# WU-CVGL/CasualHDRSplat

Hardware: AMD Instinct MI355X
Metric: train-step images/sec (fwd+bwd raster) @ 1M Gaussians 1080p (higher is better)
Workload: dtype f32; 1 GPU; c3: 1000000 Gaussians, 1920x1080, SH degree 3, HDR radiance + CRF tone-map, 1 pose(s)/view, 1 view(s)/step (one per GPU); num_rendered_R=6777809, R_prime=3025699, pixel_pair_evals_E=559372855, seed=0, binning=sync-free fixed capacity 1.25*R, launch=eager (one enqueue per kernel)

## Files before the change

### casualhdrsplat_amd/csrc/api.hip

```cpp
#include <stdarg.h>
#include <stdio.h>
#include <stdlib.h>
#include <string.h>
#include <time.h>
#include <unistd.h>
#include <atomic>

#include "hs_cloud.h"

namespace hs {

static thread_local char g_err[512] = "";

#ifdef HS_TESTING
int fault_injection() {
    static const int mode = [] {
        const char* e = getenv("HS_FAULT_INJECT");
        return (e && !strcmp(e, "sort_ticket")) ? 1 : (e && !strcmp(e, "stalled_chain")) ? 2 : (e && !strcmp(e, "late_block")) ? 3 : 0;
    }();
    return mode;
}
#endif

static std::atomic<int> g_sort_tickets{0};
#ifndef HS_TUNE_DEPTH_MSD_DEFAULT
#define HS_TUNE_DEPTH_MSD_DEFAULT 1
#endif
static std::atomic<int> g_depth_sort{-1};
#ifndef HS_TUNE_HIER_DEFAULT
#define HS_TUNE_HIER_DEFAULT 1
#endif

static int resolve_sorts(const hs_fwd_args& a, SortChoice* c) {
    if (a.tile_sort < 0 || a.tile_sort > HS_TILE_SORT_HIER || a.depth_sort < 0 || a.depth_sort > HS_DEPTH_SORT_COUNT ||
        a.chain_order < 0 || a.chain_order > HS_CHAIN_TICKETS || a.emission_scan < 0 || a.emission_scan > HS_EMISSION_SCAN_INSIDE ||
        a.depth_range_cap < 0 || a.depth_dist_max < -1) {
        set_error("hs_forward: sort selection out of range (tile_sort=%d depth_sort=%d chain_order=%d emission_scan=%d "
                  "depth_range_cap=%d depth_dist_max=%d; see hs_fwd_args in hdrsplat.h)", a.tile_sort, a.depth_sort,
                  a.chain_order, a.emission_scan, a.depth_range_cap, a.depth_dist_max);
        return HS_EINVAL;
    }
    const hs_dims& d = a.dims;
    const int64_t I = (int64_t)d.P * d.n_poses;
    const int64_t gx = (d.W + kTile - 1) / kTile, gy = (d.H + kTile - 1) / kTile;
    const bool can_count = HS_TUNE_COUNT_SORT && count_sort_fits(I, gx * gy * d.n_poses, d.capacity);
    const bool can_hier = hier_fits(I, gx, gy, d.n_poses, d.capacity);
    if (a.tile_sort == HS_TILE_SORT_RADIX) c->tile_sort = kTileSortRadix;
    else if (a.tile_sort == HS_TILE_SORT_HIER && can_hier) c->tile_sort = kTileSortHier;
    else if (a.tile_sort == HS_TILE_SORT_COUNT) c->tile_sort = can_count ? kTileSortCount : kTileSortRadix;
    else if (can_count) c->tile_sort = kTileSortCount;
    else c->tile_sort = (HS_TUNE_HIER_DEFAULT && can_hier) ? kTileSortHier : kTileSortRadix;
    if (!depth_msd_fits(I) || a.depth_sort == HS_DEPTH_SORT_PASSES) c->depth_sort = kDepthSortLsd;
    else if (a.depth_sort == HS_DEPTH_SORT_COUNT) c->depth_sort = kDepthSortMsd;
    else {
        const int v = g_depth_sort.load(std::memory_order_relaxed);
        c->depth_sort = v >= 0 ? v : (HS_TUNE_DEPTH_MSD_DEFAULT ? kDepthSortMsd : kDepthSortLsd);
    }
    c->tickets = a.chain_order ? a.chain_order == HS_CHAIN_TICKETS : g_sort_tickets.load(std::memory_order_relaxed) != 0;
    c->scan_in_emission = a.emission_scan ? a.emission_scan == HS_EMISSION_SCAN_INSIDE : (I >= (2 << 20) && !c->tickets);
    c->range_cap = a.depth_range_cap == 0 ? kMsdCap : (a.depth_range_cap < 64 ? 64 : (a.depth_range_cap > kMsdCap ? kMsdCap : a.depth_range_cap));
    c->dist_max = a.depth_dist_max == 0 ? 16 : (a.depth_dist_max < 0 ? 0 : (a.depth_dist_max > 16 ? 16 : a.depth_dist_max));
    return HS_OK;
}

static uint32_t frame_tag_seed() {
    uint64_t x = (uint64_t)getpid() * 0x9E3779B97F4A7C15ull ^ (uint64_t)time(nullptr) * 0xBF58476D1CE4E5B9ull;
    x ^= x >> 31; x *= 0x94D049BB133111EBull; x ^= x >> 29;
    return (uint32_t)x | 0x80000000u;
}
static std::atomic<uint32_t> g_frame_tag{frame_tag_seed()};
static uint32_t next_frame_tag() {
    uint32_t t;
    do { t = g_frame_tag.fetch_add(1u, std::memory_order_relaxed) + 1u; } while (t == 0u);
    return t;
}

void set_error(const char* fmt, ...) {
    va_list ap;
    va_start(ap, fmt);
    vsnprintf(g_err, sizeof g_err, fmt, ap);
    va_end(ap);
}

int64_t crf_partial_floats(int K, int64_t HW, int n_poses);
int64_t pose_partial_floats(int P, int N);

static int plan(const hs_dims& d, hs_sizes* sz, hs_layout* L) {
    if (d.P < 0 || d.W <= 0 || d.H <= 0 || d.n_poses < 1 || d.capacity < 0 || d.M < 0 || d.crf_K < 0 || d.crf_K > 4096 ||
        d.crf_K == 1 || d.n_poses > kMaxPoses) {
        set_error("hs_plan: bad dims P=%d W=%d H=%d N=%d capacity=%lld", d.P, d.W, d.H, d.n_poses, (long long)d.capacity);
        return HS_EINVAL;
    }
    if (d.n_frames < 0 || d.n_frames > d.n_poses || (d.n_frames > 1 && d.n_poses % d.n_frames != 0)) {
        set_error("hs_plan: n_frames=%d must lie in [0, n_poses=%d] and divide n_poses", d.n_frames, d.n_poses);
        return HS_EINVAL;
    }
    const int F = frames_of(d), npf = d.n_poses / F;
    const int64_t I = (int64_t)d.P * d.n_poses;
    const int64_t gx = (d.W + kTile - 1) / kTile, gy = (d.H + kTile - 1) / kTile;
    const int64_t vtiles = gx * gy * d.n_poses;
    if (I >= (1ll << 30) || vtiles >= (1ll << 31) || d.capacity >= (1ll << 30) || gx * gy >= (1ll << 22)) {
        set_error("hs_plan: problem too large (instances and binning capacity must stay below 2^30, tiles per pose below 2^22)");
        return HS_EINVAL;
    }
    const int64_t HW = (int64_t)d.W * d.H;
    hs_layout l;
    int64_t o = 0;
    auto carve = [&o](int64_t bytes) { int64_t at = o; o = align_up(o + bytes, 256); return at; };
    l.counters = carve(sizeof(hs_counters));
    l.rec = carve(I * kRecFloats * 4);
    l.depth = carve(I * 4);
    l.radii = carve(I * 4);
    l.tiles_touched = carve(I * 4);
    l.offsets = carve(I * 4);
    l.cov3D = carve((int64_t)d.P * 6 * 4);
    l.clamped = carve(I);
    l.scan_spine = carve(((I + 255) / 256 + 1) * 4);
    l.binfo = carve(I * 8);
    sz->geom_bytes = o;
    o = 0;
    l.keys_sorted = carve(2 * align_up(d.capacity * 4, 256));
    l.point_list = l.keys_sorted + align_up(d.capacity * 4, 256);
    l.pairs_tmp = carve(d.capacity * 8);
    l.ranges = carve(vtiles * 8);
    l.sort_tmp = carve(sort_tmp_bytes(I));
    l.depth_ws = carve(depth_ws_words(I) * 4);
    l.depth_pairs = carve(2 * I * 8);
    l.inst_sorted = carve(I * 4);
    l.offs_sorted = carve(I * 4);
    l.pair_sort_tmp = carve(emit_scan_words(I) * 4 + sort_tmp_bytes(d.capacity));
    l.pair_flags = carve(d.capacity);
    l.pair_act = carve(d.capacity);
    l.tile_matrix = carve(count_matrix_words(I, vtiles, d.capacity) * 4);
    l.hier_ws = carve(hier_ws_words(I, gx, gy, d.n_poses, d.capacity) * 4);
    sz->binning_bytes = o;
    o = 0;
    l.final_T = carve(HW * d.n_poses * 4);
    l.n_contrib = carve(HW * d.n_poses * 4);
    l.pose_hdr = carve(HW * 3 * 4 * (d.n_poses + (npf > 1 ? F : 0)));
    l.tile_work = carve(vtiles * 4);
    l.tile_order = carve(vtiles * 4);
    sz->image_bytes = o;
    o = 0;
    l.pair_grads = carve(d.capacity * kPairFloats * 4);
    l.crf_partials = carve(crf_partial_floats(d.crf_K, HW, d.n_poses) * 4);
    l.inst_grads = carve(I * kInstFloats * 4);
    l.pose_partials = carve(pose_partial_floats(d.P, d.n_poses) * 4);
    sz->bwd_bytes = o;
    if (L) *L = l;
    return HS_OK;
}

static int debug_sync(int flags, hipStream_t s, const char* stage) {
    if (!(flags & HS_FLAG_DEBUG)) return HS_OK;
    const hipError_t e = hipStreamSynchronize(s);
    if (e != hipSuccess) {
        set_error("debug: stage `%s` failed: %s", stage, hipGetErrorString(e));
        return HS_EHIP;
    }
    return HS_OK;
}

static int check_common(const hs_dims& d, const float* means3D, const float* shs, const float* colors,
                        const float* scales, const float* rots, const float* cov, const float* view,
                        const float* proj, const float* campos, const float* bg, const char* who) {
    if (!means3D || !view || !proj || !campos || !bg) { set_error("%s: null required pointer", who); return HS_EINVAL; }
    if ((shs == nullptr) == (colors == nullptr)) { set_error("%s: provide exactly one of shs / colors_precomp", who); return HS_EINVAL; }
    const bool sr = scales && rots;
    if (sr == (cov != nullptr) || ((scales == nullptr) != (rots == nullptr))) {
        set_error("%s: provide exactly one of (scales, rotations) / cov3D_precomp", who);
        return HS_EINVAL;
    }
    if (shs) {
        if (d.M > 32) {
            set_error("%s: M=%d SH coefficients per channel; at most 32 are supported", who, d.M);
            return HS_EINVAL;
        }
        if (d.sh_degree < 0 || d.sh_degree > 3 || (d.sh_degree + 1) * (d.sh_degree + 1) > d.M) {
            set_error("%s: sh_degree %d needs %d coefficients, M=%d", who, d.sh_degree, (d.sh_degree + 1) * (d.sh_degree + 1), d.M);
            return HS_EINVAL;
        }
    }
    if (rots && ((uintptr_t)rots & 15)) { set_error("%s: rotations must be 16-byte aligned", who); return HS_EINVAL; }
    return HS_OK;
}

static int check_flags(int flags, const char* who) {
    if ((flags & HS_FLAG_RADIANCE_EXP) && (flags & HS_FLAG_RADIANCE_SOFTPLUS)) {
        set_error("%s: HS_FLAG_RADIANCE_EXP and HS_FLAG_RADIANCE_SOFTPLUS are mutually exclusive", who);
        return HS_EINVAL;
    }
    return HS_OK;
}

static int check_loss_shape(int32_t planes, int32_t H, int32_t W, float lambda, const char* who) {
    if (planes < 1 || H < 1 || W < 1 || (int64_t)planes * H * W >= (1ll << 31)) {
        set_error("%s: bad shape planes=%d H=%d W=%d (each >= 1, planes * H * W < 2^31)", who, planes, H, W);
        return HS_EINVAL;
    }
    if (!(lambda >= 0.0f && lambda <= 1.0f)) {
        set_error("%s: lambda_dssim=%g outside [0, 1]", who, (double)lambda);
        return HS_EINVAL;
    }
    return HS_OK;
}

static int check_activate_tensor(const char* who, const char* name, const void* key, const void* const* need, const char* const* need_names, int n) {
    if (!key) return HS_OK;
    if (check_aligned(who, key, name, 4)) return HS_EINVAL;
    for (int i = 0; i < n; ++i) {
        if (!need[i]) { set_error("%s: %s is given but %s is NULL", who, name, need_names[i]); return HS_EINVAL; }
        if (check_aligned(who, need[i], need_names[i], 4)) return HS_EINVAL;
    }
    return HS_OK;
}

}

using namespace hs;

extern "C" {

int hs_version(void) { return HS_VERSION; }

const char* hs_last_error(void) { return g_err; }

int hs_plan(const hs_dims* dims, hs_sizes* sizes, hs_layout* layout) {
    if (!dims || !sizes) { set_error("hs_plan: null argument"); return HS_EINVAL; }
    return plan(*dims, sizes, layout);
}

int hs_max_frames(void) { return kMaxPoses; }

#ifdef HS_TESTING
HS_API uint32_t hs_test_next_frame_tag(void) {
    const uint32_t t = g_frame_tag.load(std::memory_order_relaxed) + 1u;
    return t == 0u ? 1u : t;
}
#endif

int hs_forward(const hs_fwd_args* a, void* hip_stream) {
    if (!a) { set_error("hs_forward: null args"); return HS_EINVAL; }
    hipStream_t s = (hipStream_t)hip_stream;
    hs_sizes sz; hs_layout L;
    int rc = plan(a->dims, &sz, &L);
    if (rc) return rc;
    if ((rc = check_flags(a->flags, "hs_forward"))) return rc;
    SortChoice sort;
    if ((rc = resolve_sorts(*a, &sort))) return rc;
    if (a->dims.P > 0) {
        rc = check_common(a->dims, a->means3D, a->shs, a->colors_precomp, a->scales, a->rotations, a->cov3D_precomp,
                          a->viewmatrices, a->projmatrices, a->camposes, a->bg, "hs_forward");
        if (rc) return rc;
        if (!a->opacities || ((a->stages & HS_STAGE_PREPROCESS) && !a->radii)) {
            set_error("hs_forward: null opacities/radii");
            return HS_EINVAL;
        }
    }
    if (!a->geom || !a->bg) { set_error("hs_forward: null geom/bg"); return HS_EINVAL; }
    if ((a->flags & HS_FLAG_HDR) && (!a->exposure || !a->crf_table || a->crf_K < 2 || a->crf_K > 4096 || !(a->crf_umax > a->crf_umin))) {
        set_error("hs_forward: HDR needs exposure, crf_table, 2 <= crf_K <= 4096 and umax > umin");
        return HS_EINVAL;
    }
    if ((a->flags & HS_FLAG_HDR) && a->dims.crf_K != a->crf_K) {
        set_error("hs_forward: dims.crf_K (%d, sizes the workspaces) differs from crf_K (%d)", a->dims.crf_K, a->crf_K);
        return HS_EINVAL;
    }
    if (((uintptr_t)a->geom & 255) || ((uintptr_t)a->binning & 255) || ((uintptr_t)a->image & 255)) {
        set_error("hs_forward: workspaces must be 256-byte aligned");
        return HS_EINVAL;
    }
    if (a->dims.P == 0) {
        const int64_t gx0 = (a->dims.W + kTile - 1) / kTile, gy0 = (a->dims.H + kTile - 1) / kTile;
        const bool bin = (a->stages & HS_STAGE_BIN) && !(a->stages & HS_STAGE_PREPROCESS_ONLY) && a->binning;
        rc = launch_empty_frame((a->stages & HS_STAGE_PREPROCESS) ? (hs_counters*)((char*)a->geom + L.counters) : nullptr,
                                bin ? (uint2*)((char*)a->binning + L.ranges) : nullptr, gx0 * gy0 * a->dims.n_poses,
                                bin ? (uint32_t*)a->counters_host : nullptr, (const hs_counters*)((char*)a->geom + L.counters), s);
        if (rc) return rc;
    }
    const uint32_t frame_tag = ((a->stages & HS_STAGE_PREPROCESS) && (a->stages & HS_STAGE_BIN) && a->binning) ? next_frame_tag() : 0u;
    if ((a->stages & HS_STAGE_PREPROCESS) && a->dims.P > 0) {
        rc = launch_preprocess_fwd(*a, L, s, frame_tag);
        if (rc) return rc;
        if ((rc = debug_sync(a->flags, s, "preprocess"))) return rc;
        if (!(a->stages & HS_STAGE_BIN)) {
            rc = launch_scan(*a, L, s);
            if (rc) return rc;
        }
    }
    if ((a->stages & HS_STAGE_BIN) && !(a->stages & HS_STAGE_PREPROCESS_ONLY)) {
        if (!a->binning) { set_error("hs_forward: null binning workspace"); return HS_EINVAL; }
        if (a->dims.P > 0) {
            rc = launch_binning(*a, L, sort, s, frame_tag);
            if (rc) return rc;
            if ((rc = debug_sync(a->flags, s, "binning"))) return rc;
        }
    }
    if ((a->stages & HS_STAGE_OFFSETS) && a->dims.P > 0) {
        rc = launch_scan(*a, L, s);
        if (rc) return rc;
        if ((rc = launch_cov3d(*a, L, s))) return rc;
        if (a->binning && a->dims.capacity > 0)
            if ((rc = launch_tile_keys(*a, L, s))) return rc;
    }
    if (a->stages & HS_STAGE_RENDER) {
        if (!a->binning || !a->image || !a->out_color) { set_error("hs_forward: null binning/image/out_color"); return HS_EINVAL; }
        rc = launch_render_fwd(*a, L, s);
        if (rc) return rc;
        if ((rc = debug_sync(a->flags, s, "render forward"))) return rc;
    }
    return HS_OK;
}

int hs_backward(const hs_bwd_args* a, void* hip_stream) {
    if (!a) { set_error("hs_backward: null args"); return HS_EINVAL; }
    hipStream_t s = (hipStream_t)hip_stream;
    hs_sizes sz; hs_layout L;
    int rc = plan(a->dims, &sz, &L);
    if (rc) return rc;
    if ((rc = check_flags(a->flags, "hs_backward"))) return rc;
    if (frames_of(a->dims) > 1 && (a->dL_dout_alpha || a->dL_dout_invdepth)) {
        set_error("hs_backward: dL_dout_alpha / dL_dout_invdepth are per-image gradients and are not supported with n_frames=%d",
                  a->dims.n_frames);
        return HS_EINVAL;
    }
    rc = check_common(a->dims, a->means3D, a->shs, a->colors_precomp, a->scales, a->rotations, a->cov3D_precomp,
                      a->viewmatrices, a->projmatrices, a->camposes, a->bg, "hs_backward");
    if (rc) return rc;
    if (!a->geom || !a->binning || !a->image || !a->bwd || !a->dL_dout_color) {
        set_error("hs_backward: null workspace or dL_dout_color");
        return HS_EINVAL;
    }
    if ((a->flags & HS_FLAG_HDR) && (!a->exposure || !a->crf_table || a->crf_K < 2 || a->crf_K > 4096 || a->dims.crf_K != a->crf_K)) {
        set_error("hs_backward: HDR needs exposure, crf_table and dims.crf_K == crf_K");
        return HS_EINVAL;
    }
    const int npose_out = (a->dL_dviewmatrices != nullptr) + (a->dL_dprojmatrices != nullptr) + (a->dL_dcamposes != nullptr);
    if (npose_out != 0 && npose_out != 3) {
        set_error("hs_backward: pose gradients need dL_dviewmatrices, dL_dprojmatrices and dL_dcamposes together");
        return HS_EINVAL;
    }
    const int ndens = (a->densify_grad_accum != nullptr) + (a->densify_denom != nullptr) + (a->densify_max_radii != nullptr);
    if (ndens != 0 && ndens != 3) {
        set_error("hs_backward: densification statistics need grad_accum, denom and max_radii together");
        return HS_EINVAL;
    }
    if (a->g_begin != 0 || a->g_end != 0) {
        if (a->g_begin < 0 || a->g_end < a->g_begin || a->g_end > a->dims.P || (a->g_begin & 127) ||
            (a->stages & ~HS_BWD_PROJECT)) {
            set_error("hs_backward: [g_begin, g_end) = [%d, %d) needs 0 <= g_begin <= g_end <= P, g_begin a multiple of 128, "
                      "and stages == HS_BWD_PROJECT", a->g_begin, a->g_end);
            return HS_EINVAL;
        }
    }
    if (a->dims.P == 0) return HS_OK;
    const bool crf_in_tail = HS_TUNE_CRF_IN_RENDER_TAIL && (a->stages & HS_BWD_RENDER) && (a->stages & HS_BWD_CRF) &&
                             !(a->flags & HS_FLAG_DEBUG) && a->crf_K <= 1024;
    if (a->stages & HS_BWD_RENDER) {
        rc = launch_render_bwd(*a, L, s, nullptr, nullptr, crf_in_tail);
        if (rc) return rc;
        if ((rc = debug_sync(a->flags, s, "render backward"))) return rc;
    }
    CrfReduce crf_reduce{nullptr, 0, 0, 0, nullptr, nullptr, 0};
    const bool sums_follow = (a->stages & (HS_BWD_PREPROCESS | HS_BWD_SEGSUM)) != 0 && !(a->flags & HS_FLAG_DEBUG);
    if (a->stages & HS_BWD_CRF) {
        rc = launch_crf_bwd(*a, L, s, sums_follow ? &crf_reduce : nullptr, crf_in_tail);
        if (rc) return rc;
        if ((rc = debug_sync(a->flags, s, "CRF gradient"))) return rc;
    }
    if (a->stages & (HS_BWD_PREPROCESS | HS_BWD_SEGSUM | HS_BWD_PROJECT)) {
        const bool whole = (a->stages & HS_BWD_PREPROCESS) != 0;
        rc = launch_preprocess_bwd(*a, L, s, whole || (a->stages & HS_BWD_SEGSUM), whole || (a->stages & HS_BWD_PROJECT),
                                   crf_reduce.nblocks ? &crf_reduce : nullptr);
        if (rc) return rc;
        if ((rc = debug_sync(a->flags, s, "preprocess backward"))) return rc;
    }
    return HS_OK;
}

int hs_depth_sort(int mode) {
    if (mode >= 0) hs::g_depth_sort.store(mode ? 1 : 0, std::memory_order_relaxed);
    const int v = hs::g_depth_sort.load(std::memory_order_relaxed);
    return v >= 0 ? v : (HS_TUNE_DEPTH_MSD_DEFAULT ? 1 : 0);
}

int hs_sort_tickets(int enable) {
    if (enable >= 0) hs::g_sort_tickets.store(enable ? 1 : 0, std::memory_order_relaxed);
    return hs::g_sort_tickets.load(std::memory_order_relaxed);
}

int hs_mark_visible(int32_t P, const float* means3D, const float* viewmatrix, uint8_t* visible, void* hip_stream) {
    if (P < 0 || (P > 0 && (!means3D || !viewmatrix || !visible))) { set_error("hs_mark_visible: bad argument"); return HS_EINVAL; }
    if (P == 0) return HS_OK;
    return launch_mark_visible(P, means3D, viewmatrix, visible, (hipStream_t)hip_stream);
}

int hs_sh_backward_views(int32_t P, int32_t M, int32_t sh_degree, int32_t V, const float* means3D, const float* camposes,
                         const float* dL_dview_colors, float* dL_dshs, void* hip_stream) {
    if (P < 0 || V < 1 || sh_degree < 0 || sh_degree > 3 || M < (sh_degree + 1) * (sh_degree + 1) || M > 16 ||
        (P > 0 && (!means3D || !camposes || !dL_dview_colors || !dL_dshs))) {
        set_error("hs_sh_backward_views: bad argument");
        return HS_EINVAL;
    }
    if (P == 0) return HS_OK;
    return launch_sh_backward_views(P, M, sh_degree, V, means3D, camposes, dL_dview_colors, dL_dshs, (hipStream_t)hip_stream);
}

int hs_spline_poses(int32_t n_knots, int32_t n_times, int32_t kind, const float* delta, const float* base_w2c,
                    const float* times, float* w2c, float* jacobian, int32_t* segment, void* hip_stream) {
    if (n_times < 0 || (kind != 0 && kind != 1) || n_knots < (kind == 1 ? 4 : 2) ||
        (n_times > 0 && (!delta || !base_w2c || !times || !w2c || !jacobian || !segment))) {
        set_error("hs_spline_poses: bad argument (kind 0 = linear needs >= 2 knots, 1 = cubic >= 4)");
        return HS_EINVAL;
    }
    if (n_times == 0) return HS_OK;
    return launch_spline_poses(n_knots, n_times, kind, delta, base_w2c, times, w2c, jacobian, segment, (hipStream_t)hip_stream);
}

int hs_render_stats(const hs_fwd_args* fwd, const hs_bwd_args* bwd, uint64_t* stats, uint64_t* bwd_timeline, void* hip_stream) {
    if ((!fwd && !bwd) || !stats) { set_error("hs_render_stats: null argument"); return HS_EINVAL; }
    hipStream_t s = (hipStream_t)hip_stream;
    hs_sizes sz; hs_layout L;
    if (fwd) {
        int rc = plan(fwd->dims, &sz, &L);
        if (rc) return rc;
        if (!fwd->geom || !fwd->binning || !fwd->image || !fwd->out_color || !fwd->bg) {
            set_error("hs_render_stats: forward args need geom/binning/image/out_color/bg");
            return HS_EINVAL;
        }
        if (fwd->dims.P > 0 && (rc = launch_render_fwd(*fwd, L, s, (unsigned long long*)stats))) return rc;
    }
    if (bwd) {
        int rc = plan(bwd->dims, &sz, &L);
        if (rc) return rc;
        if (!bwd->geom || !bwd->binning || !bwd->image || !bwd->bwd || !bwd->dL_dout_color || !bwd->bg) {
            set_error("hs_render_stats: backward args need geom/binning/image/bwd/dL_dout_color/bg");
            return HS_EINVAL;
        }
        if (bwd->dims.P > 0 && (rc = launch_render_bwd(*bwd, L, s, (unsigned long long*)stats, (unsigned long long*)bwd_timeline))) return rc;
    }
    return HS_OK;
}

int64_t hs_loss_workspace_bytes(int32_t planes, int32_t H, int32_t W, int32_t with_partials) {
    if (check_loss_shape(planes, H, W, 0.0f, "hs_loss_workspace_bytes")) return HS_EINVAL;
    const int64_t pairs = align_up(loss_pair_count(planes, H, W) * 16, 256);
    return pairs + (with_partials ? (int64_t)12 * planes * H * W : 0);
}

int hs_photometric_loss(const hs_loss_args* a, void* hip_stream) {
    if (!a) { set_error("hs_photometric_loss: null args"); return HS_EINVAL; }
    int rc = check_loss_shape(a->planes, a->H, a->W, a->lambda_dssim, "hs_photometric_loss");
    if (rc) return rc;
    if (!a->image || !a->target || !a->workspace || !a->out) {
        set_error("hs_photometric_loss: null image/target/workspace/out");
        return HS_EINVAL;
    }
    if ((uintptr_t)a->workspace & 255) { set_error("hs_photometric_loss: workspace must be 256-byte aligned"); return HS_EINVAL; }
    return launch_loss_fwd(*a, (hipStream_t)hip_stream);
}

int hs_photometric_loss_backward(const hs_loss_args* a, void* hip_stream) {
    if (!a) { set_error("hs_photometric_loss_backward: null args"); return HS_EINVAL; }
    int rc = check_loss_shape(a->planes, a->H, a->W, a->lambda_dssim, "hs_photometric_loss_backward");
    if (rc) return rc;
    if (!a->image || !a->target || !a->partials || !a->dL_dloss || !a->dL_dimage) {
        set_error("hs_photometric_loss_backward: null image/target/partials/dL_dloss/dL_dimage");
        return HS_EINVAL;
    }
    return launch_loss_bwd(*a, (hipStream_t)hip_stream);
}

int hs_activate(const hs_activate_args* a, void* hip_stream) {
    const char* who = "hs_activate";
    if (check_args(who, a) || check_rows(who, "P", a->P)) return HS_EINVAL;
    int rc;
    if (a->P == 0) return HS_OK;
    const void* o[] = {a->opacities}; const char* on[] = {"opacities"};
    const void* s[] = {a->scales}; const char* sn[] = {"scales"};
    const void* r[] = {a->rotations}; const char* rn[] = {"rotations"};
    if ((rc = check_activate_tensor(who, "opacity_raw", a->opacity_raw, o, on, 1))) return rc;
    if ((rc = check_activate_tensor(who, "scales_raw", a->scales_raw, s, sn, 1))) return rc;
    if ((rc = check_activate_tensor(who, "rotations_raw", a->rotations_raw, r, rn, 1))) return rc;
    return launch_activate_fwd(*a, (hipStream_t)hip_stream);
}

int hs_activate_backward(const hs_activate_args* a, void* hip_stream) {
    const char* who = "hs_activate_backward";
    if (check_args(who, a) || check_rows(who, "P", a->P)) return HS_EINVAL;
    int rc;
    if (a->g_begin < 0 || a->g_begin > a->g_end || a->g_end > a->P) {
        set_error("%s: rows [g_begin=%lld, g_end=%lld) are not inside [0, P=%lld]", who, (long long)a->g_begin, (long long)a->g_end,
                  (long long)a->P);
        return HS_EINVAL;
    }
    if (a->g_begin == a->g_end) return HS_OK;
    const void* o[] = {a->opacities}; const char* on[] = {"opacities"};
    const void* s[] = {a->scales}; const char* sn[] = {"scales"};
    const void* r[] = {a->rotations, a->rotations_raw}; const char* rn[] = {"rotations", "rotations_raw"};
    if ((rc = check_activate_tensor(who, "dL_dopacities", a->dL_dopacities, o, on, 1))) return rc;
    if ((rc = check_activate_tensor(who, "dL_dscales", a->dL_dscales, s, sn, 1))) return rc;
    if ((rc = check_activate_tensor(who, "dL_drotations", a->dL_drotations, r, rn, 2))) return rc;
    return launch_activate_bwd(*a, (hipStream_t)hip_stream);
}

int64_t hs_sort_tmp_bytes(int64_t n) { return sort_tmp_bytes(n) + 256 + 2 * align_up(n * 8, 256) + 2 * align_up(n * 4, 256); }

int hs_sort_pairs(const uint64_t* keys_in, const uint32_t* vals_in, uint64_t* keys_out, uint32_t* vals_out,
                  int64_t n, int32_t nbits, void* tmp, void* hip_stream) {
    if (n < 0 || n >= (1ll << 30) || nbits < 1 || nbits > 64 || (n > 0 && (!keys_in || !vals_in || !keys_out || !vals_out || !tmp))) {
        set_error("hs_sort_pairs: bad argument");
        return HS_EINVAL;
    }
    if (n == 0) return HS_OK;
    hipStream_t s = (hipStream_t)hip_stream;
    char* t = (char*)tmp;
    uint32_t* n_dev = (uint32_t*)t;
    uint32_t* fail_word = n_dev + 1; t += 256;
    uint64_t* kb = (uint64_t*)t; t += align_up(n * 8, 256);
    uint32_t* vb = (uint32_t*)t; t += align_up(n * 4, 256);
    uint64_t* ka = (uint64_t*)t; t += align_up(n * 8, 256);
    uint32_t* va = (uint32_t*)t; t += align_up(n * 4, 256);
    HS_HIP_CHECK(hipMemsetD32Async((hipDeviceptr_t)n_dev, (int)(uint32_t)n, 1, s));
    HS_HIP_CHECK(hipMemsetD32Async((hipDeviceptr_t)fail_word, 0, 1, s));
    HS_HIP_CHECK(hipMemcpyAsync(ka, keys_in, (size_t)n * 8, hipMemcpyDeviceToDevice, s));
    HS_HIP_CHECK(hipMemcpyAsync(va, vals_in, (size_t)n * 4, hipMemcpyDeviceToDevice, s));
    int rc = launch_radix_sort(ka, va, kb, vb, n_dev, n, nbits, t, fail_word, s);
    if (rc) return rc;
    const bool in_a = sort_passes(nbits) % 2 == 0;
    HS_HIP_CHECK(hipMemcpyAsync(keys_out, in_a ? ka : kb, (size_t)n * 8, hipMemcpyDeviceToDevice, s));
    HS_HIP_CHECK(hipMemcpyAsync(vals_out, in_a ? va : vb, (size_t)n * 4, hipMemcpyDeviceToDevice, s));
    return HS_OK;
}

}
```

### casualhdrsplat_amd/csrc/hs_common.h

```cpp
#pragma once
#include <hip/hip_runtime.h>
#include <stdint.h>

#include "../../include/hdrsplat.h"

#if defined(__HIP_DEVICE_COMPILE__) && !defined(__gfx950__)
#error "libhdrsplat is written for gfx950 (MI355X) only: build with --offload-arch=gfx950"
#endif

namespace hs {

void set_error(const char* fmt, ...);

#define HS_HIP_CHECK(expr)                                                                         \
    do {                                                                                           \
        hipError_t e_ = (expr);                                                                    \
        if (e_ != hipSuccess) {                                                                    \
            ::hs::set_error("%s failed: %s (%s:%d)", #expr, hipGetErrorString(e_), __FILE__, __LINE__); \
            return HS_EHIP;                                                                        \
        }                                                                                          \
    } while (0)
#define HS_LAUNCH_CHECK() HS_HIP_CHECK(hipGetLastError())

#ifndef HS_TUNE_CRF_IN_RENDER_TAIL
#define HS_TUNE_CRF_IN_RENDER_TAIL 1
#endif

#ifndef HS_TUNE_COUNT_SORT
#define HS_TUNE_COUNT_SORT 1
#endif

constexpr int kTile = HS_TILE;
constexpr int kRecF4 = 4;
constexpr int kPairF4 = 4;
constexpr int kInstF4 = 4;
constexpr int kRecFloats = 4 * kRecF4;
constexpr int kPairFloats = 4 * kPairF4;
constexpr int kInstFloats = 4 * kInstF4;
constexpr int kSortBlock = 256;
constexpr int kDepthBins = 512, kDepthDigitBits = 9;
#ifndef HS_TUNE_DEPTH_ITEMS
#define HS_TUNE_DEPTH_ITEMS 8
#endif
constexpr int kDepthSortItems = HS_TUNE_DEPTH_ITEMS, kDepthSortLook = 8;
constexpr int kPairSortItems = 16, kPairSortLook = 8;
constexpr int kU64SortItems = 16;
constexpr int kDepthTile = kDepthSortItems * kDepthBins, kPairTile = kPairSortItems * kSortBlock, kU64Tile = kU64SortItems * kSortBlock;
static_assert(kPairTile == kU64Tile && kDepthTile >= kPairTile, "the scratch of every sort is sized for the smallest tile");
constexpr int kSortTileMin = kPairTile;

static inline int64_t align_up(int64_t v, int64_t a) { return (v + a - 1) / a * a; }
static inline int ceil_div(int64_t a, int64_t b) { return (int)((a + b - 1) / b); }
constexpr int kMaxPoses = 21845;
static inline int frames_of(const hs_dims& d) { return d.n_frames > 1 ? d.n_frames : 1; }

static inline int tile_bits(uint32_t n) {
    int b = 0;
    while (n) { ++b; n >>= 1; }
    return b;
}

int launch_preprocess_fwd(const hs_fwd_args& a, const hs_layout& L, hipStream_t s, uint32_t frame_tag);
int launch_scan(const hs_fwd_args& a, const hs_layout& L, hipStream_t s);
int launch_cov3d(const hs_fwd_args& a, const hs_layout& L, hipStream_t s);
struct SortChoice;
int launch_binning(const hs_fwd_args& a, const hs_layout& L, const SortChoice& sort, hipStream_t s, uint32_t frame_tag);
int launch_empty_frame(hs_counters* clear, uint2* ranges, int64_t ntiles, uint32_t* counters_host, const hs_counters* counters,
                       hipStream_t s);
int launch_render_fwd(const hs_fwd_args& a, const hs_layout& L, hipStream_t s, unsigned long long* stats = nullptr);
int launch_render_bwd(const hs_bwd_args& a, const hs_layout& L, hipStream_t s, unsigned long long* stats = nullptr,
                      unsigned long long* timeline = nullptr, bool crf_in_tail = false);
int render_stats_count();
struct CrfReduce;
int launch_crf_bwd(const hs_bwd_args& a, const hs_layout& L, hipStream_t s, CrfReduce* defer, bool in_render_tail = false);
int launch_preprocess_bwd(const hs_bwd_args& a, const hs_layout& L, hipStream_t s, bool segsum, bool project,
                          const CrfReduce* crf_reduce);
int launch_mark_visible(int P, const float* means3D, const float* view, uint8_t* vis, hipStream_t s);
int launch_spline_poses(int J, int T, int kind, const float* delta, const float* base, const float* times, float* w2c,
                        float* jac, int* seg, hipStream_t s);
int launch_sh_backward_views(int P, int M, int deg, int V, const float* means3D, const float* camposes,
                             const float* view_colors, float* d_shs, hipStream_t s);
int64_t loss_pair_count(int planes, int H, int W);
int launch_loss_fwd(const hs_loss_args& a, hipStream_t s);
int launch_loss_bwd(const hs_loss_args& a, hipStream_t s);
int launch_activate_fwd(const hs_activate_args& a, hipStream_t s);
int launch_activate_bwd(const hs_activate_args& a, hipStream_t s);

constexpr int kGhistCopies = 16;
constexpr int kGhistWords = kGhistCopies * 8 * 256;
constexpr int kTicketWords = 128, kDepthBitsAt = 32, kDepthBitsCopies = 16, kDepthBitsWords = 4 * kDepthBitsCopies;
static_assert(kDepthBitsAt >= 8 && kDepthBitsAt % 2 == 0 && kDepthBitsAt + kDepthBitsWords <= kTicketWords, "depth bits live in the ticket row");
__host__ __device__ inline int64_t sweep_pass_words(int64_t nblk, int bins = 256) { return nblk * bins; }
static inline int64_t sort_scratch_words(int64_t n, int passes, int tile, int bins = 256) {
    return n > 0 ? kGhistWords + kTicketWords + (int64_t)passes * sweep_pass_words((n + tile - 1) / tile, bins) : 0;
}
static inline int64_t depth_scratch_words(int64_t I) { return sort_scratch_words(I, 4, kDepthTile, kDepthBins); }
int64_t sort_tmp_bytes(int64_t n);
constexpr int kMsdBits = 12, kMsdBuckets = 1 << kMsdBits;
#ifndef HS_TUNE_MSD_RANGE
#define HS_TUNE_MSD_RANGE 2048
#endif
constexpr int kMsdRange = HS_TUNE_MSD_RANGE, kMsdCap = 4096;
#ifndef HS_TUNE_MSD_SMALL_RANGE
#define HS_TUNE_MSD_SMALL_RANGE 512
#endif
static inline int depth_msd_range(int64_t I) { return I <= (1 << 18) ? HS_TUNE_MSD_SMALL_RANGE : kMsdRange; }
static inline bool depth_msd_fits(int64_t I) { return I > 0 && I < (2 << 20); }
static inline int depth_msd_tile(int64_t I) { return I <= (1 << 18) ? 1024 : 4096; }
static inline int64_t depth_msd_rows(int64_t I) { return (I + depth_msd_tile(I) - 1) / depth_msd_tile(I); }
static inline int64_t depth_ws_words(int64_t I) {
    return depth_msd_fits(I) ? depth_msd_rows(I) * (kMsdBuckets / 2 + kMsdBuckets + 1) + kMsdBuckets : 0;
}
enum DepthSort { kDepthSortLsd = 0, kDepthSortMsd = 1 };
static inline int64_t emit_scan_words(int64_t I) { return 2 * ((I + 255) / 256 + 2) / 64 * 64 + 64; }
static inline int64_t pair_scratch_words(int64_t I, int64_t capacity, int passes) {
    return emit_scan_words(I) + sort_scratch_words(capacity, passes, kPairSortItems * kSortBlock);
}
int launch_radix_sort(uint64_t* k0, uint32_t* v0, uint64_t* k1, uint32_t* v1, const uint32_t* n_dev,
                      int64_t n_launch, int nbits, void* tmp, uint32_t* fail_word, hipStream_t s, bool zeroed = false);
#ifdef HS_TESTING
int fault_injection();
#else
constexpr int fault_injection() { return 0; }
#endif
static inline int sort_passes(int nbits) { return (nbits + 7) / 8; }
constexpr int kCountTilesMax = 4096;
constexpr int64_t kCountMatrixMax = 1ll << 21;
static inline bool count_sort_fits(int64_t I, int64_t vtiles, int64_t capacity) {
    return capacity > 0 && I > 0 && vtiles <= kCountTilesMax && ((I + 255) / 256) * vtiles <= kCountMatrixMax;
}
static inline int64_t count_matrix_words(int64_t I, int64_t vtiles, int64_t capacity) {
    return count_sort_fits(I, vtiles, capacity) ? 2 * ((I + 255) / 256) * vtiles + vtiles : 0;
}
constexpr int kSuper = 8;
constexpr int kHierStMax = 2048;
constexpr int kHierChunkMin = 512, kHierChunkMax = 1024, kHierRoundsMax = kHierChunkMax / 4 / 64;
static inline int hier_chunk(int64_t I) { return I >= (2ll << 20) ? kHierChunkMax : kHierChunkMin; }
constexpr int kHierCopies = 16;
static inline int64_t hier_super_tiles(int64_t gx, int64_t gy, int64_t n_poses) {
    return ((gx + kSuper - 1) / kSuper) * ((gy + kSuper - 1) / kSuper) * n_poses;
}
static inline bool hier_fits(int64_t I, int64_t gx, int64_t gy, int64_t n_poses, int64_t capacity) {
    return capacity > 0 && I > 0 && hier_super_tiles(gx, gy, n_poses) <= kHierStMax;
}
struct HierWs {
    int64_t nst, chunks_max;
    int64_t st_count, tile_total, zero_words, tile_start, coarse_first, chunk_first, desc, counts, words;
    HierWs(int64_t gx, int64_t gy, int64_t n_poses, int64_t capacity) {
        nst = hier_super_tiles(gx, gy, n_poses);
        chunks_max = (capacity + kHierChunkMin - 1) / kHierChunkMin + nst;
        const int64_t nst_pad = (nst + 63) / 64 * 64;
        int64_t o = 64;
        st_count = o; o += kHierCopies * nst_pad;
        tile_total = o; o += nst * 64;
        zero_words = o;
        tile_start = o; o += nst * 64;
        coarse_first = o; o += nst_pad + 64;
        chunk_first = o; o += nst_pad + 64;
        desc = o; o += chunks_max * 4;
        counts = o; o += chunks_max * 64 * 2;
        words = o;
    }
    int64_t nst_pad() const { return (nst + 63) / 64 * 64; }
};
static inline int64_t hier_ws_words(int64_t I, int64_t gx, int64_t gy, int64_t n_poses, int64_t capacity) {
    return hier_fits(I, gx, gy, n_poses, capacity) ? HierWs(gx, gy, n_poses, capacity).words : 0;
}
enum TileSort { kTileSortRadix = 0, kTileSortCount = 1, kTileSortHier = 2 };
struct SortChoice {
    int tile_sort;
    int depth_sort;
    bool tickets;
    bool scan_in_emission;
    int range_cap;
    int dist_max;
};
int launch_tile_keys(const hs_fwd_args& a, const hs_layout& L, hipStream_t s);

__device__ __forceinline__ void tagged_or(unsigned long long* p, uint32_t tag, uint32_t bits) {
    unsigned long long old = __hip_atomic_load(p, __ATOMIC_RELAXED, __HIP_MEMORY_SCOPE_AGENT);
    for (;;) {
        const unsigned long long cur = (uint32_t)(old >> 32) == tag ? old : ((unsigned long long)tag << 32);
        const unsigned long long nw = cur | bits;
        if (nw == old) return;
        const unsigned long long prev = atomicCAS(p, old, nw);
        if (prev == old) return;
        old = prev;
    }
}
template <int CTRL, int ROW_MASK = 0xF>
__device__ __forceinline__ float dpp_f32(float v) {
    return __int_as_float(__builtin_amdgcn_update_dpp(0, __float_as_int(v), CTRL, ROW_MASK, 0xF, false));
}
__device__ __forceinline__ float wave_sum_hi_f32(float v) {
    v += dpp_f32<0xB1>(v);
    v += dpp_f32<0x4E>(v);
    v += dpp_f32<0x141>(v);
    v += dpp_f32<0x140>(v);
    v += dpp_f32<0x142, 0xA>(v);
    v += dpp_f32<0x143, 0xC>(v);
    return v;
}

struct CrfReduce {
    const float* partials; int bx, planes, K; float* d_table; float* d_exposure;
    int nblocks;
    int F;
};
__device__ __forceinline__ void crf_reduce_block(const CrfReduce& c, int block) {
    const int K = c.K;
    const int i = block * 4 + (threadIdx.x >> 6);
    const int lane = threadIdx.x & 63;
    if (i >= 3 * K + c.F) return;
    const bool expo = i >= 3 * K;
    const int ch = expo ? 0 : i / K, k = expo ? K : i - ch * K;
    float acc = 0.f;
    const int frame_rows = (c.planes / c.F) * c.bx;
    const int nrows = expo ? frame_rows : (c.planes / 3) * c.bx;
    const int row0 = expo ? (i - 3 * K) * frame_rows : 0;
    for (int r = lane; r < nrows; r += 64) {
        const int row = expo ? row0 + r : ((r / c.bx) * 3 + ch) * c.bx + (r % c.bx);
        acc += c.partials[(int64_t)row * (K + 1) + k];
    }
    acc = wave_sum_hi_f32(acc);
    if (lane == 63) {
        if (!expo) { if (c.d_table) c.d_table[i] = acc; }
        else if (c.d_exposure) c.d_exposure[i - 3 * K] = acc;
    }
}

template <int CTRL, int ROW_MASK = 0xF>
__device__ __forceinline__ uint32_t dpp_u32(uint32_t v) {
    return (uint32_t)__builtin_amdgcn_update_dpp(0, (int)v, CTRL, ROW_MASK, 0xF, false);
}
__device__ __forceinline__ uint32_t wave_or_hi(uint32_t v) {
    v |= dpp_u32<0xB1>(v);
    v |= dpp_u32<0x4E>(v);
    v |= dpp_u32<0x141>(v);
    v |= dpp_u32<0x140>(v);
    v |= dpp_u32<0x142, 0xA>(v);
    v |= dpp_u32<0x143, 0xC>(v);
    return v;
}
__device__ __forceinline__ void depth_bits_accumulate2(uint32_t o_in, uint32_t nz_in, unsigned long long* bits, uint32_t tag,
                                                       uint32_t* s_two ) {
    const uint32_t o = wave_or_hi(o_in), nz = wave_or_hi(nz_in);
    if ((threadIdx.x & 63) == 63) { if (o) atomicOr(&s_two[0], o); if (nz) atomicOr(&s_two[1], nz); }
    __syncthreads();
    if (threadIdx.x < 2 && s_two[threadIdx.x])
        tagged_or(bits + 2 * (blockIdx.x % kDepthBitsCopies) + threadIdx.x, tag, s_two[threadIdx.x]);
}
__device__ __forceinline__ void depth_bits_accumulate(uint32_t key, bool visible, unsigned long long* bits, uint32_t tag,
                                                      uint32_t* s_two ) {
    depth_bits_accumulate2(visible ? key : 0u, visible ? ~key : 0u, bits, tag, s_two);
}
__device__ __forceinline__ float radiance_dact(int act, float col, bool was_clamped) {
    if (act == 1) return col;
    if (act == 2) return -expm1f(-col);
    return was_clamped ? 0.f : 1.f;
}

struct SegsumArgs {
    int64_t I;
    const uint32_t* inst_sorted; const uint32_t* offs_sorted;
    const float4* pair_grads; const uint8_t* pair_flags; float4* inst_grads; const hs_counters* counters;
    const int* radii_inst; const uint8_t* clamped; float* view_colors; const float4* rec; int act;
};
__device__ __forceinline__ void pair_segsum_body(const SegsumArgs& a, int64_t t) {
    const int64_t i = t >> 2;
    const int q = (int)(t & 3);
    const bool valid = i < a.I && !a.counters->overflow;
    const uint32_t beg = valid ? (i == 0 ? 0u : a.offs_sorted[i - 1]) : 0u;
    const uint32_t end = valid ? a.offs_sorted[i] : 0u;
    float r[10] = {0.f, 0.f, 0.f, 0.f, 0.f, 0.f, 0.f, 0.f, 0.f, 0.f};
    for (uint32_t s = beg + q; s < end; s += 8) {
        const bool two = s + 4 < end;
        const bool f0 = a.pair_flags[s] != 0;
        const bool f1 = two && a.pair_flags[s + 4] != 0;
        float4 a0 = make_float4(0.f, 0.f, 0.f, 0.f), a1 = a0, b0 = a0, b1 = a0;
        float2 a2 = make_float2(0.f, 0.f), b2 = a2;
        if (f0) {
            a0 = a.pair_grads[kPairF4 * (int64_t)s + 0];
            a1 = a.pair_grads[kPairF4 * (int64_t)s + 1];
            a2 = reinterpret_cast<const float2*>(a.pair_grads + kPairF4 * (int64_t)s + 2)[0];
        }
        if (f1) {
            b0 = a.pair_grads[kPairF4 * (int64_t)(s + 4) + 0];
            b1 = a.pair_grads[kPairF4 * (int64_t)(s + 4) + 1];
            b2 = reinterpret_cast<const float2*>(a.pair_grads + kPairF4 * (int64_t)(s + 4) + 2)[0];
        }
        r[0] += a0.x; r[1] += a0.y; r[2] += a0.z; r[3] += a0.w;
        r[4] += a1.x; r[5] += a1.y; r[6] += a1.z; r[7] += a1.w;
        r[8] += a2.x; r[9] += a2.y;
        r[0] += b0.x; r[1] += b0.y; r[2] += b0.z; r[3] += b0.w;
        r[4] += b1.x; r[5] += b1.y; r[6] += b1.z; r[7] += b1.w;
        r[8] += b2.x; r[9] += b2.y;
    }
#pragma unroll
    for (int k = 0; k < 10; ++k) {
        r[k] += __shfl_xor(r[k], 1);
        r[k] += __shfl_xor(r[k], 2);
    }
    if (i < a.I && q == 0) {
        const int64_t inst = a.counters->overflow >= 2u ? i : (int64_t)a.inst_sorted[i];
        float4* o = a.inst_grads + kInstF4 * inst;
        o[0] = make_float4(r[0], r[1], r[2], r[3]);
        o[1] = make_float4(r[4], r[5], r[6], r[7]);
        o[2] = make_float4(r[8], r[9], 0.f, 0.f);
        if constexpr (kInstF4 == 4) o[3] = make_float4(0.f, 0.f, 0.f, 0.f);
        if (a.view_colors) {
            const uint8_t cl = a.clamped[inst];
            const bool on = a.radii_inst[inst] > 0;
            float col[3] = {0.f, 0.f, 0.f};
            if (a.act != 0 && on) {
                const float4 rb = a.rec[kRecF4 * inst + 1];
                col[0] = rb.z; col[1] = rb.w; col[2] = reinterpret_cast<const float*>(a.rec + kRecF4 * inst + 2)[0];
            }
            a.view_colors[3 * inst + 0] = on ? radiance_dact(a.act, col[0], cl & 1) * r[6] : 0.f;
            a.view_colors[3 * inst + 1] = on ? radiance_dact(a.act, col[1], cl & 2) * r[7] : 0.f;
            a.view_colors[3 * inst + 2] = on ? radiance_dact(a.act, col[2], cl & 4) * r[8] : 0.f;
        }
    }
}

__device__ __forceinline__ float xform_row(const float* m, int i, float x, float y, float z) {
    return ((m[i] * x + m[4 + i] * y) + m[8 + i] * z) + m[12 + i];
}

}
```

### casualhdrsplat_amd/csrc/render.hip

```cpp
#include "hs_common.h"

namespace hs {

namespace {

constexpr float kAlphaMin = 1.0f / 255.0f;
constexpr float kAlphaMax = 0.99f;
constexpr float kTmin = 0.0001f;
constexpr float kLogEps = 1e-8f;


enum {
    kStBwdTrips = 0,
    kStBwdEmpty = 1,
    kStBwdActivePix = 2,
    kStBwdCulled = 3,
    kStBwdHist = 4,
    kStBwdStaged = 10,
    kStBwdBatches = 11,
    kStFwdTrips = 12, kStFwdEmpty = 13, kStFwdActivePix = 14, kStFwdCulled = 15, kStFwdStaged = 16, kStFwdBatches = 17,
    kStCount = 24
};
struct WaveStats {
    unsigned long long v[kStCount];
    __device__ __forceinline__ void clear() {
#pragma unroll
        for (int i = 0; i < kStCount; ++i) v[i] = 0;
    }
    __device__ __forceinline__ void flush(unsigned long long* dst) const {
        if ((threadIdx.x & 63) == 0) {
#pragma unroll
            for (int i = 0; i < kStCount; ++i)
                if (v[i]) atomicAdd(dst + i, v[i]);
        }
    }
};

template <int CTRL, int ROW_MASK = 0xF>
__device__ __forceinline__ float dpp(float v) {
    return __int_as_float(__builtin_amdgcn_update_dpp(0, __float_as_int(v), CTRL, ROW_MASK, 0xF, false));
}
__device__ __forceinline__ float wave_sum_hi(float v) {
    v += dpp<0xB1>(v);
    v += dpp<0x4E>(v);
    v += dpp<0x141>(v);
    v += dpp<0x140>(v);
    v += dpp<0x142, 0xA>(v);
    v += dpp<0x143, 0xC>(v);
    return v;
}
__device__ __forceinline__ float halve16(float x, float y) {
    auto r = __builtin_amdgcn_permlane16_swap(__float_as_uint(x), __float_as_uint(y), false, false);
    return __uint_as_float(r[0]) + __uint_as_float(r[1]);
}
template <bool TEN>
__device__ __forceinline__ void reduce_in_rows(const float* g, float g9, float& w0, float& w1, float& w2) {
    float z0, z1, z2, z3, z4;
    if constexpr (TEN) {
        asm("s_nop 1\n\t"
            "v_add_f32_dpp %3, %9, %9 row_shr:8 row_mask:0xf bank_mask:0xc\n\t"
            "v_add_f32_dpp %3, %8, %8 row_shl:8 row_mask:0xf bank_mask:0x3\n\t"
            "v_add_f32_dpp %4, %11, %11 row_shr:8 row_mask:0xf bank_mask:0xc\n\t"
            "v_add_f32_dpp %4, %10, %10 row_shl:8 row_mask:0xf bank_mask:0x3\n\t"
            "v_add_f32_dpp %5, %13, %13 row_shr:8 row_mask:0xf bank_mask:0xc\n\t"
            "v_add_f32_dpp %5, %12, %12 row_shl:8 row_mask:0xf bank_mask:0x3\n\t"
            "v_add_f32_dpp %6, %15, %15 row_shr:8 row_mask:0xf bank_mask:0xc\n\t"
            "v_add_f32_dpp %6, %14, %14 row_shl:8 row_mask:0xf bank_mask:0x3\n\t"
            "v_add_f32_dpp %7, %17, %17 row_shr:8 row_mask:0xf bank_mask:0xc\n\t"
            "v_add_f32_dpp %7, %16, %16 row_shl:8 row_mask:0xf bank_mask:0x3\n\t"
            "v_add_f32_dpp %0, %4, %4 row_shr:4 row_mask:0xf bank_mask:0xa\n\t"
            "v_add_f32_dpp %0, %3, %3 row_shl:4 row_mask:0xf bank_mask:0x5\n\t"
            "v_add_f32_dpp %1, %6, %6 row_shr:4 row_mask:0xf bank_mask:0xa\n\t"
            "v_add_f32_dpp %1, %5, %5 row_shl:4 row_mask:0xf bank_mask:0x5\n\t"
            "v_add_f32_dpp %2, %7, %7 row_shr:4 row_mask:0xf bank_mask:0xa\n\t"
            "v_add_f32_dpp %2, %7, %7 row_shl:4 row_mask:0xf bank_mask:0x5\n\t"
            "s_nop 1"
            : "=&v"(w0), "=&v"(w1), "=&v"(w2), "=&v"(z0), "=&v"(z1), "=&v"(z2), "=&v"(z3), "=&v"(z4)
            : "v"(g[0]), "v"(g[1]), "v"(g[2]), "v"(g[3]), "v"(g[4]), "v"(g[5]), "v"(g[6]), "v"(g[7]), "v"(g[8]), "v"(g9));
    } else {
        asm("s_nop 1\n\t"
            "v_add_f32_dpp %3, %9, %9 row_shr:8 row_mask:0xf bank_mask:0xc\n\t"
            "v_add_f32_dpp %3, %8, %8 row_shl:8 row_mask:0xf bank_mask:0x3\n\t"
            "v_add_f32_dpp %4, %11, %11 row_shr:8 row_mask:0xf bank_mask:0xc\n\t"
            "v_add_f32_dpp %4, %10, %10 row_shl:8 row_mask:0xf bank_mask:0x3\n\t"
            "v_add_f32_dpp %5, %13, %13 row_shr:8 row_mask:0xf bank_mask:0xc\n\t"
            "v_add_f32_dpp %5, %12, %12 row_shl:8 row_mask:0xf bank_mask:0x3\n\t"
            "v_add_f32_dpp %6, %15, %15 row_shr:8 row_mask:0xf bank_mask:0xc\n\t"
            "v_add_f32_dpp %6, %14, %14 row_shl:8 row_mask:0xf bank_mask:0x3\n\t"
            "v_add_f32_dpp %7, %16, %16 row_ror:8 row_mask:0xf bank_mask:0xf\n\t"
            "v_add_f32_dpp %0, %4, %4 row_shr:4 row_mask:0xf bank_mask:0xa\n\t"
            "v_add_f32_dpp %0, %3, %3 row_shl:4 row_mask:0xf bank_mask:0x5\n\t"
            "v_add_f32_dpp %1, %6, %6 row_shr:4 row_mask:0xf bank_mask:0xa\n\t"
            "v_add_f32_dpp %1, %5, %5 row_shl:4 row_mask:0xf bank_mask:0x5\n\t"
            "v_add_f32_dpp %2, %7, %7 row_ror:4 row_mask:0xf bank_mask:0xf\n\t"
            "s_nop 1"
            : "=&v"(w0), "=&v"(w1), "=&v"(w2), "=&v"(z0), "=&v"(z1), "=&v"(z2), "=&v"(z3), "=&v"(z4)
            : "v"(g[0]), "v"(g[1]), "v"(g[2]), "v"(g[3]), "v"(g[4]), "v"(g[5]), "v"(g[6]), "v"(g[7]), "v"(g[8]));
    }
}
__device__ __forceinline__ float reduce_in_quads(float t) {
    asm("s_nop 1\n\t"
        "v_add_f32_dpp %0, %0, %0 quad_perm:[1,0,3,2] row_mask:0xf bank_mask:0xf\n\t"
        "s_nop 1\n\t"
        "v_add_f32_dpp %0, %0, %0 quad_perm:[2,3,0,1] row_mask:0xf bank_mask:0xf"
        : "+v"(t));
    return t;
}

template <bool TEN>
__device__ __forceinline__ void group_reduce(const float* g, float g9, int xor16_addr, float& t0, float& t1) {
    float w0, w1, w2;
    reduce_in_rows<TEN>(g, g9, w0, w1, w2);
    const float u0 = halve16(w0, w1);
    const float u1 = w2 + __int_as_float(__builtin_amdgcn_ds_bpermute(xor16_addr, __float_as_int(w2)));
    t0 = reduce_in_quads(u0);
    t1 = reduce_in_quads(u1);
}

__device__ __forceinline__ int mask_prefix(uint64_t m) {
    return (int)__builtin_amdgcn_mbcnt_hi((uint32_t)(m >> 32), __builtin_amdgcn_mbcnt_lo((uint32_t)m, 0u));
}

__device__ __forceinline__ uint32_t wave_max_u32(uint32_t v) {
#pragma unroll
    for (int d = 32; d >= 1; d >>= 1) v = max(v, (uint32_t)__shfl_xor((int)v, d));
    return v;
}

struct Crf {
    const float* table;
    int K;
    float umin, umax, dt;
};

__device__ __forceinline__ void crf_locate(const Crf& c, float Hv, int& i, float& f, float& xv, bool& interior) {
    xv = Hv * c.dt;
    const float u = __logf(fmaxf(xv, kLogEps));
    float s = (u - c.umin) / (c.umax - c.umin) * (float)(c.K - 1);
    bool in = true;
    if (!(s > 0.f)) { s = 0.f; in = false; }
    if (s >= (float)(c.K - 1)) { s = (float)(c.K - 1); in = false; }
    i = (int)floorf(s);
    if (i > c.K - 2) i = c.K - 2;
    f = s - (float)i;
    interior = in && (xv > kLogEps);
}
__device__ __forceinline__ float crf_eval(const Crf& c, int ch, float Hv) {
    int i; float f, xv; bool in;
    crf_locate(c, Hv, i, f, xv, in);
    const float* t = c.table + ch * c.K;
    return t[i] * (1.f - f) + t[i + 1] * f;
}
__device__ __forceinline__ float crf_grad_H(const Crf& c, int ch, float Hv, float g) {
    int i; float f, xv; bool in;
    crf_locate(c, Hv, i, f, xv, in);
    if (!in) return 0.f;
    const float* t = c.table + ch * c.K;
    const float scale = (float)(c.K - 1) / (c.umax - c.umin);
    return g * (t[i + 1] - t[i]) * scale / xv * c.dt;
}

constexpr float kLog2e = 1.4426950408889634f;

typedef float f2 __attribute__((ext_vector_type(2)));

#ifndef HS_NO_OPSEL_ASM
__device__ __forceinline__ f2 pk_fma_hi(f2 pair, f2 w, f2 acc) {
    asm("v_pk_fma_f32 %0, %1, %2, %0 op_sel:[1,0,0] op_sel_hi:[1,1,1]" : "+v"(acc) : "v"(pair), "v"(w));
    return acc;
}
__device__ __forceinline__ f2 pk_mul_hi(f2 pair, f2 w) {
    f2 r;
    asm("v_pk_mul_f32 %0, %1, %2 op_sel:[1,0] op_sel_hi:[1,1]" : "=v"(r) : "v"(pair), "v"(w));
    return r;
}
#else
__device__ __forceinline__ f2 pk_fma_hi(f2 pair, f2 w, f2 acc) { return acc + f2{pair.y, pair.y} * w; }
__device__ __forceinline__ f2 pk_mul_hi(f2 pair, f2 w) { return f2{pair.y, pair.y} * w; }
#endif

__device__ __forceinline__ void scale_entry(float4& a, float4& b) {
    a.z *= -0.5f * kLog2e; a.w *= -kLog2e; b.x *= -0.5f * kLog2e;
}

template <int WIDTH>
__device__ __forceinline__ bool block_may_touch(const float4 a, const float4 b, float sx, float sy) {
    const float A2 = a.z, B2 = a.w, C2 = b.x, o = b.y;
    if (!(o >= kAlphaMin)) return false;
    if (!(A2 < 0.f && C2 < 0.f && 4.f * A2 * C2 - B2 * B2 > 0.f)) return true;
    const float thr = -(__log2f(255.f * o) * 1.0001f + 0.05f);
    const float dx_lo = a.x - (sx + (float)(WIDTH - 1)), dx_hi = a.x - sx, dy_lo = a.y - (sy + 7.f), dy_hi = a.y - sy;
    const float dx_e = fminf(fmaxf(0.f, dx_lo), dx_hi);
    const float dy_e = fminf(fmaxf(0.f, dy_lo), dy_hi);
    const float dy_s = fminf(fmaxf(-0.5f * B2 * dx_e / C2, dy_lo), dy_hi);
    const float dx_s = fminf(fmaxf(-0.5f * B2 * dy_e / A2, dx_lo), dx_hi);
    const float p1 = dx_e * (A2 * dx_e + B2 * dy_s) + C2 * dy_s * dy_s;
    const float p2 = dx_s * (A2 * dx_s + B2 * dy_e) + C2 * dy_e * dy_e;
    return fmaxf(p1, p2) >= thr;
}

__device__ __forceinline__ void lane_pixels(int lane, int sx, int sy, int& px, int& py0) {
    px = sx + 8 * (lane >> 5) + (lane & 7);
    py0 = sy + 2 * ((lane >> 3) & 3);
}

struct RenderFwd {
    int W, H, gx, ntiles, N, flags;
    const uint2* ranges; const uint32_t* point_list; const float4* rec; const float* bg;
    float* out_color; float* out_hdr; float* final_T; uint32_t* n_contrib; float* pose_hdr;
    float* out_invdepth;
    Crf crf;
    const float* exposure;
    unsigned long long* stats;
    unsigned long long* timeline;
    uint8_t* pair_act;
    uint32_t* tile_work;
};

constexpr int kBatch = 128;

__device__ __forceinline__ int xcd_strip_tile(int b, int nb, int gx) {
    constexpr int kXcd = 8, kRows = 2;
    const int x = b % kXcd, k = b / kXcd;
    const int per = nb / kXcd, rem = nb % kXcd;
    int p = x * per + min(x, rem) + k;
    const int rows = nb / gx;
    const int nstrips = (rows + kRows - 1) / kRows;
    const int strip_tiles = kRows * gx;
    const int last_short = nstrips * strip_tiles - nb;
    int c = 0;
    for (; c < kXcd - 1; ++c) {
        const int ns = (nstrips - c + kXcd - 1) / kXcd;
        const int nt = ns * strip_tiles - (((nstrips - 1) % kXcd) == c ? last_short : 0);
        if (p < nt) break;
        p -= nt;
    }
    const int s_local = p / strip_tiles, r = p - s_local * strip_tiles;
    return (c + kXcd * s_local) * strip_tiles + r;
}

__device__ __forceinline__ float hs_exp2(float x) { return __builtin_amdgcn_exp2f(x); }

struct PixF {
    float T, C0, C1, C2, D;
    uint32_t last;
};
constexpr int kFcmpOGE = 3, kFcmpOLE = 5;
struct PairF {
    f2 T, C0, C1, C2, D;
    uint32_t last0, last1;
};
template <bool DEPTH>
__device__ __forceinline__ uint64_t blend_fwd_pair(PairF& s, uint64_t& done0, uint64_t& done1, f2 pw, f2 alpha, float r,
                                                   float g, float b, float invd, uint32_t idx1, int* n_pixels = nullptr) {
    const uint64_t valid0 = ~done0 & __builtin_amdgcn_fcmpf(pw.x, 0.f, kFcmpOLE) &
                            __builtin_amdgcn_fcmpf(alpha.x, kAlphaMin, kFcmpOGE);
    const uint64_t valid1 = ~done1 & __builtin_amdgcn_fcmpf(pw.y, 0.f, kFcmpOLE) &
                            __builtin_amdgcn_fcmpf(alpha.y, kAlphaMin, kFcmpOGE);
    const f2 one = {1.f, 1.f};
    const f2 test_T = s.T * (one - alpha);
    const uint64_t cont0 = valid0 & __builtin_amdgcn_fcmpf(test_T.x, kTmin, kFcmpOGE);
    const uint64_t cont1 = valid1 & __builtin_amdgcn_fcmpf(test_T.y, kTmin, kFcmpOGE);
    done0 |= valid0 ^ cont0;
    done1 |= valid1 ^ cont1;
    const bool upd0 = __builtin_amdgcn_inverse_ballot_w64(cont0), upd1 = __builtin_amdgcn_inverse_ballot_w64(cont1);
    const f2 aT = alpha * s.T;
    const f2 w = {upd0 ? aT.x : 0.f, upd1 ? aT.y : 0.f};
    const f2 rr = {r, r}, bb = {b, b};
    s.C0 += rr * w; s.C1 = pk_fma_hi(f2{r, g}, w, s.C1); s.C2 += bb * w;
    if constexpr (DEPTH) { const f2 dd = {invd, invd}; s.D += dd * w; }
    s.T = f2{upd0 ? test_T.x : s.T.x, upd1 ? test_T.y : s.T.y};
    s.last0 = upd0 ? idx1 : s.last0;
    s.last1 = upd1 ? idx1 : s.last1;
    if (n_pixels) *n_pixels = __popcll(cont0) + __popcll(cont1);
    return cont0 | cont1;
}

__device__ __forceinline__ void write_pixel_fwd(const RenderFwd& p, const PixF& st, int pose, int px, int py) {
    const int64_t HW = (int64_t)p.H * p.W;
    const int64_t pix = (int64_t)py * p.W + px;
    p.final_T[(int64_t)pose * HW + pix] = st.T;
    p.n_contrib[(int64_t)pose * HW + pix] = st.last;
    const float H0 = st.C0 + st.T * p.bg[0], H1 = st.C1 + st.T * p.bg[1], H2 = st.C2 + st.T * p.bg[2];
    const bool hdr = p.flags & HS_FLAG_HDR;
    if (p.pose_hdr) {
        float* ph = p.pose_hdr + (int64_t)pose * 3 * HW;
        ph[pix] = H0; ph[HW + pix] = H1; ph[2 * HW + pix] = H2;
    }
    if (p.N == 1) {
        float* const oc = p.out_color + (int64_t)pose * 3 * HW;
        if (hdr) {
            Crf c = p.crf;
            c.dt = p.exposure[pose];
            if (p.out_hdr) { float* const oh = p.out_hdr + (int64_t)pose * 3 * HW; oh[pix] = H0; oh[HW + pix] = H1; oh[2 * HW + pix] = H2; }
            oc[pix] = crf_eval(c, 0, H0);
            oc[HW + pix] = crf_eval(c, 1, H1);
            oc[2 * HW + pix] = crf_eval(c, 2, H2);
        } else {
            oc[pix] = H0; oc[HW + pix] = H1; oc[2 * HW + pix] = H2;
        }
    }
}

constexpr int kFwdEntF = 12;

template <bool DEPTH, bool STATS>
__global__ void __launch_bounds__(kBatch) __attribute__((amdgpu_waves_per_eu((DEPTH || STATS) ? 1 : 7)))
render_fwd_kernel(RenderFwd p) {
    constexpr int KB = kBatch;
    constexpr int kEnt = kFwdEntF * 4;
    constexpr int kSentinel = KB * kEnt;
    constexpr int kListLen = KB + 8;
    __shared__ __attribute__((aligned(16))) float s_ent[(KB + 1) * kFwdEntF];
    __shared__ int s_alive[2][2];
    __shared__ uint16_t s_list[2][2][kListLen];
    __shared__ uint8_t s_taken[2][2][KB];
    __shared__ uint32_t s_work[2];

    const int vt = xcd_strip_tile(blockIdx.x, gridDim.x, p.gx);
    const int pose = vt / p.ntiles;
    const int tile = vt - pose * p.ntiles;
    const int tx = tile % p.gx, ty = tile / p.gx;
    const int wave = threadIdx.x >> 6, lane = threadIdx.x & 63;
    const int grp = lane >> 5;
    const int sx = tx * kTile, sy = ty * kTile + wave * 8;
    int px, py0;
    lane_pixels(lane, sx, sy, px, py0);
    const int py1 = py0 + 1;
    const bool in0 = px < p.W && py0 < p.H, in1 = px < p.W && py1 < p.H;
    const float pxf = (float)px;
    const f2 pyf = {(float)py0, (float)py1};
    const float sxf = (float)sx, syf = (float)sy;

    const uint2 range = p.ranges[vt];
    const int n = (int)(range.y - range.x);

    PairF ps;
    ps.T = f2{1.f, 1.f};
    ps.C0 = ps.C1 = ps.C2 = ps.D = f2{0.f, 0.f};
    ps.last0 = ps.last1 = 0;
    uint64_t done0 = __builtin_amdgcn_ballot_w64(!in0), done1 = __builtin_amdgcn_ballot_w64(!in1);

    float4 ra = make_float4(0.f, 0.f, 0.f, 0.f), rb = ra;
    float rcb = 0.f, rdepth = 1.f;
    if ((int)threadIdx.x < n) {
        const uint32_t id = p.point_list[range.x + threadIdx.x];
        const float4* r = p.rec + kRecF4 * (int64_t)id;
        ra = r[0]; rb = r[1]; rcb = reinterpret_cast<const float*>(r + 2)[0];
        if constexpr (DEPTH) rdepth = reinterpret_cast<const float*>(r + 2)[1];
    }
    WaveStats ws;
    if constexpr (STATS) ws.clear();
    const char* const ent = reinterpret_cast<const char*>(s_ent);
    float* const my_ent = s_ent + threadIdx.x * kFwdEntF;
    const uint16_t* const my_list = s_list[wave][grp];
    if (threadIdx.x < kFwdEntF) s_ent[KB * kFwdEntF + threadIdx.x] = 0.f;
    auto flush_activity = [&](int base_prev, int cnt_prev) {
        const int t = threadIdx.x;
        if (t < cnt_prev)
            p.pair_act[(int64_t)range.x + base_prev + t] = (uint8_t)(s_taken[0][0][t] | s_taken[0][1][t] | s_taken[1][0][t] | s_taken[1][1][t]);
        s_taken[0][0][t] = 0; s_taken[0][1][t] = 0; s_taken[1][0][t] = 0; s_taken[1][1][t] = 0;
    };
    auto walk = [&](int i0, int i1, int base48) -> uint32_t {
        uint32_t act_lo = 0u, act_hi = 0u;
        uint32_t pos = 0u;
        const uint32_t npos = (uint32_t)(i1 - i0);
        const uint16_t* lp = my_list + i0;
        auto trip = [&]() {
            const int jb = (int)*lp++;
            const char* e = ent + jb;
            const float4 a = *reinterpret_cast<const float4*>(e);
            const float4 b = *reinterpret_cast<const float4*>(e + 16);
            const float2 c = *reinterpret_cast<const float2*>(e + 32);
            const float dx = a.x - pxf;
            const f2 dy = a.y - pyf;
            const float t = a.z * dx * dx, u = a.w * dx;
            const f2 pw = dy * (b.x * dy + u) + t;
            const float al0 = fminf(kAlphaMax, b.y * hs_exp2(pw.x));
            const float al1 = fminf(kAlphaMax, b.y * hs_exp2(pw.y));
            const uint32_t idx48 = (uint32_t)(base48 + jb + kEnt);
            int n_pix = 0;
            const uint64_t took = blend_fwd_pair<DEPTH>(ps, done0, done1, pw, f2{al0, al1}, b.z, b.w, c.x, DEPTH ? c.y : 0.f, idx48,
                                                        STATS ? &n_pix : nullptr);
            if constexpr (STATS) ws.v[kStFwdActivePix] += n_pix;
#pragma clang diagnostic push
#pragma clang diagnostic ignored "-Winline-asm"
            asm("s_mov_b32 m0, %2\n\t"
                "v_writelane_b32 %0, %3, m0\n\t"
                "v_writelane_b32 %1, %4, m0\n\t"
                "s_add_u32 %2, %2, 1"
                : "+v"(act_lo), "+v"(act_hi), "+s"(pos) : "s"((uint32_t)took), "s"((uint32_t)(took >> 32)) : "scc", "m0");
#pragma clang diagnostic pop
            if constexpr (STATS) { ws.v[kStFwdTrips] += 1; ws.v[kStFwdEmpty] += took == 0ull; }
        };
        if (npos >= 2u) {
            do {
                trip();
                trip();
            } while (pos + 2u <= npos && (done0 & done1) != ~0ull);
        }
        if (pos + 1u == npos && (done0 & done1) != ~0ull) trip();
        return (act_lo != 0u ? 1u : 0u) | (act_hi != 0u ? 4u : 0u);
    };
    s_taken[0][0][threadIdx.x] = 0; s_taken[0][1][threadIdx.x] = 0; s_taken[1][0][threadIdx.x] = 0; s_taken[1][1][threadIdx.x] = 0;
    uint32_t n_taken = 0;
    int it = 0, base = 0;
    for (; base < n; base += KB, ++it) {
        const uint64_t fin = done0 & done1;
        const bool wave_alive = fin != ~0ull;
        if (lane == 0) s_alive[it & 1][wave] = wave_alive;
        __syncthreads();
        if (it > 0) flush_activity(base - KB, KB);
        if (!(s_alive[it & 1][0] | s_alive[it & 1][1])) break;
        const int cnt = min(KB, n - base);
        if constexpr (STATS) { if (wave == 0) { ws.v[kStFwdStaged] += cnt; ws.v[kStFwdBatches] += 1; } }
        if ((int)threadIdx.x < cnt) {
            scale_entry(ra, rb);
            reinterpret_cast<float4*>(my_ent)[0] = ra;
            reinterpret_cast<float4*>(my_ent)[1] = rb;
            reinterpret_cast<float2*>(my_ent)[4] = make_float2(rcb, DEPTH ? 1.f / rdepth : 0.f);
        }
        if (base + KB + (int)threadIdx.x < n) {
            const uint32_t id = p.point_list[range.x + base + KB + threadIdx.x];
            const float4* r = p.rec + kRecF4 * (int64_t)id;
            ra = r[0]; rb = r[1]; rcb = reinterpret_cast<const float*>(r + 2)[0];
            if constexpr (DEPTH) rdepth = reinterpret_cast<const float*>(r + 2)[1];
        }
        __syncthreads();
        if (wave_alive) {
            const bool alive_g[2] = {(uint32_t)fin != 0xFFFFFFFFu, (uint32_t)(fin >> 32) != 0xFFFFFFFFu};
            int n_g[2] = {0, 0};
#pragma unroll
            for (int k = 0; k < KB / 64; ++k) {
                const int jj = k * 64 + lane;
                bool touch[2] = {false, false};
                if (jj < cnt) {
                    const float4 a = reinterpret_cast<const float4*>(s_ent + jj * kFwdEntF)[0];
                    const float4 b = reinterpret_cast<const float4*>(s_ent + jj * kFwdEntF)[1];
                    touch[0] = alive_g[0] && block_may_touch<8>(a, b, sxf, syf);
                    touch[1] = alive_g[1] && block_may_touch<8>(a, b, sxf + 8.f, syf);
                }
                if constexpr (STATS) ws.v[kStFwdCulled] += __popcll(__ballot(jj < cnt && !touch[0] && !touch[1]));
#pragma unroll
                for (int g = 0; g < 2; ++g) {
                    const uint64_t mask = __ballot(touch[g]);
                    if (touch[g]) s_list[wave][g][n_g[g] + mask_prefix(mask)] = (uint16_t)(jj * kEnt);
                    n_g[g] += __popcll(mask);
                }
            }
            const int n_t = max(n_g[0], n_g[1]);
#pragma unroll
            for (int g = 0; g < 2; ++g)
#pragma unroll
                for (int t = lane; t < kListLen; t += 64)
                    if (t >= n_g[g]) s_list[wave][g][t] = (uint16_t)kSentinel;
            const uint32_t t0 = walk(0, min(n_t, 64), base * kEnt);
            const uint32_t t1 = ((done0 & done1) != ~0ull && n_t > 64) ? walk(64, n_t, base * kEnt) : 0u;

#pragma unroll
            for (int g = 0; g < 2; ++g) {
                const uint32_t bit = 1u << (2 * g);
                if (t0 & bit) s_taken[wave][g][s_list[wave][g][lane] / kEnt] = (uint8_t)(bit << wave);
                if (t1 & bit) s_taken[wave][g][s_list[wave][g][64 + lane] / kEnt] = (uint8_t)(bit << wave);
                n_taken += (uint32_t)(__popcll(__ballot((t0 & bit) != 0u)) + __popcll(__ballot((t1 & bit) != 0u)));
            }
        }
    }
    if (it > 0 && base >= n) {
        __syncthreads();
        flush_activity(base - KB, n - (base - KB));
    }
    if (lane == 0) s_work[wave] = n_taken;
    __syncthreads();
    if (threadIdx.x == 0) p.tile_work[vt] = s_work[0] + s_work[1];
    {
        float* const o = s_ent + wave * (6 * 128);
        const int pos0 = (py0 - sy) * 16 + (px - sx), pos1 = pos0 + 16;
        o[pos0] = ps.T.x; o[pos1] = ps.T.y;
        o[128 + pos0] = __uint_as_float(ps.last0); o[128 + pos1] = __uint_as_float(ps.last1);
        o[256 + pos0] = ps.C0.x; o[256 + pos1] = ps.C0.y;
        o[384 + pos0] = ps.C1.x; o[384 + pos1] = ps.C1.y;
        o[512 + pos0] = ps.C2.x; o[512 + pos1] = ps.C2.y;
        if constexpr (DEPTH) { o[640 + pos0] = ps.D.x; o[640 + pos1] = ps.D.y; }
        const int qx = sx + (lane & 15), qy0 = sy + 2 * (lane >> 4);
        const int r0 = (qy0 - sy) * 16 + (lane & 15), r1 = r0 + 16;
        PixF s0, s1;
        s0.T = o[r0]; s0.last = __float_as_uint(o[128 + r0]) / (kFwdEntF * 4); s0.C0 = o[256 + r0]; s0.C1 = o[384 + r0]; s0.C2 = o[512 + r0];
        s1.T = o[r1]; s1.last = __float_as_uint(o[128 + r1]) / (kFwdEntF * 4); s1.C0 = o[256 + r1]; s1.C1 = o[384 + r1]; s1.C2 = o[512 + r1];
        const bool q0 = qx < p.W && qy0 < p.H, q1 = qx < p.W && qy0 + 1 < p.H;
        if (q0) write_pixel_fwd(p, s0, pose, qx, qy0);
        if (q1) write_pixel_fwd(p, s1, pose, qx, qy0 + 1);
        if constexpr (DEPTH) {
            const int64_t HW = (int64_t)p.H * p.W;
            if (q0) p.out_invdepth[(int64_t)pose * HW + (int64_t)qy0 * p.W + qx] = o[640 + r0];
            if (q1) p.out_invdepth[(int64_t)pose * HW + (int64_t)(qy0 + 1) * p.W + qx] = o[640 + r1];
        }
    }
    if constexpr (STATS) ws.flush(p.stats);
}

__global__ void __launch_bounds__(256) resolve_kernel(int64_t HW, int N, int F, int flags, float* pose_hdr, Crf crf,
                                                      const float* exposure, float* out_color, float* out_hdr) {
    const int64_t i = (int64_t)blockIdx.x * 256 + threadIdx.x;
    if (i >= (int64_t)F * 3 * HW) return;
    const int f = (int)(i / (3 * HW));
    const int64_t j = i - (int64_t)f * 3 * HW;
    const int ch = (int)(j / HW);
    const bool hdr = flags & HS_FLAG_HDR;
    if (hdr) crf.dt = exposure[f];
    float sumH = 0.f, sumL = 0.f;
    const float* planes = pose_hdr + (int64_t)f * N * 3 * HW + j;
    for (int k = 0; k < N; ++k) {
        const float Hv = planes[(int64_t)k * 3 * HW];
        sumH += Hv;
        if (hdr && !(flags & HS_FLAG_BLUR_HDR)) sumL += crf_eval(crf, ch, Hv);
    }
    const float inv = 1.f / (float)N;
    const float meanH = sumH * inv;
    pose_hdr[((int64_t)F * N + f) * 3 * HW + j] = meanH;
    if (hdr) {
        if (out_hdr) out_hdr[i] = meanH;
        out_color[i] = (flags & HS_FLAG_BLUR_HDR) ? crf_eval(crf, ch, meanH) : sumL * inv;
    } else {
        out_color[i] = meanH;
    }
}

__global__ void __launch_bounds__(1024) order_tiles_kernel(int nb, int gx, int n_static, const uint32_t* work,
                                                           uint32_t* order) {
    constexpr int kBins = 1024, kT = 1024;
    __shared__ uint32_t s_hist[kBins];
    __shared__ uint32_t s_scan[kT / 64];
    __shared__ uint32_t s_thr_bin, s_thr_take;
    const int x = blockIdx.x, t = threadIdx.x;
    const int per = nb / 8, rem = nb % 8;
    const int cnt = per + (x < rem ? 1 : 0);
    const int n_keep = n_static > x ? (n_static - x + 7) / 8 : 0;
    const int n_light = cnt - n_keep;
    int q_base = 0;
    for (int y = 0; y < x; ++y) q_base += (per + (y < rem ? 1 : 0)) - (n_static > y ? (n_static - y + 7) / 8 : 0);
    const int E = (cnt + kT - 1) / kT;
    const int k0 = t * E, k1 = min(cnt, (t + 1) * E);
    if (E > 64) {
        for (int k = k0; k < k1; ++k) order[x + 8 * k] = (uint32_t)xcd_strip_tile(x + 8 * k, nb, gx);
        return;
    }
    auto block_excl_scan = [&](uint32_t v, uint32_t* total) -> uint32_t {
        uint32_t incl = v;
#pragma unroll
        for (int d = 1; d < 64; d <<= 1) { const uint32_t u = __shfl_up(incl, d); if ((t & 63) >= d) incl += u; }
        __syncthreads();
        if ((t & 63) == 63) s_scan[t >> 6] = incl;
        __syncthreads();
        uint32_t add = 0, tot = 0;
        for (int w = 0; w < kT / 64; ++w) { const uint32_t c = s_scan[w]; if (w < (t >> 6)) add += c; tot += c; }
        *total = tot;
        return add + incl - v;
    };
    auto bin_of = [&](int k) { return (int)min((uint32_t)(kBins - 1), work[xcd_strip_tile(x + 8 * k, nb, gx)] >> 1); };
    s_hist[t] = 0;
    if (t == 0) { s_thr_bin = 0; s_thr_take = 0; }
    __syncthreads();
    for (int k = k0; k < k1; ++k) atomicAdd(&s_hist[bin_of(k)], 1u);
    __syncthreads();
    {
        uint32_t tot;
        const uint32_t h = s_hist[t];
        const uint32_t below = block_excl_scan(h, &tot);
        if (below < (uint32_t)n_light && below + h >= (uint32_t)n_light) { s_thr_bin = t; s_thr_take = (uint32_t)n_light - below; }
    }
    __syncthreads();
    const int thr = (int)s_thr_bin;
    const uint32_t take = s_thr_take;
    uint32_t in_thr = 0;
    for (int k = k0; k < k1; ++k) in_thr += bin_of(k) == thr ? 1u : 0u;
    uint32_t tot_thr;
    uint32_t thr_rank = block_excl_scan(in_thr, &tot_thr);
    uint64_t light_mask = 0;
    uint32_t kept = 0;
    for (int k = k0; k < k1; ++k) {
        const int b = bin_of(k);
        const bool light = n_light > 0 && (b < thr || (b == thr && thr_rank++ < take));
        light_mask |= (uint64_t)light << (k - k0);
        kept += !light;
    }
    uint32_t tot_kept;
    uint32_t kpos = block_excl_scan(kept, &tot_kept);
    uint32_t qpos = (uint32_t)k0 - kpos;
    for (int k = k0; k < k1; ++k) {
        const uint32_t vt = (uint32_t)xcd_strip_tile(x + 8 * k, nb, gx);
        if ((light_mask >> (k - k0)) & 1ull) order[n_static + q_base + (int)qpos++] = vt;
        else order[x + 8 * (int)kpos++] = vt;
    }
}

constexpr int kCrfPixPerWave = 1024;

struct CrfGradArgs {
    int64_t HW; int N, F, flags;
    const float* pose_hdr; Crf crf; const float* exposure; const float* dL_dcolor; float* partials;
    int bx, planes;
};

template <int NW>
__device__ __forceinline__ void crf_grad_body(const CrfGradArgs& A, const int bxi, const int plane_in,
                                              unsigned long long* const s_tab64) {
    const int64_t HW = A.HW; const int N = A.N, flags = A.flags; const float* pose_hdr = A.pose_hdr; Crf crf = A.crf;
    const float* exposure = A.exposure; const float* dL_dcolor = A.dL_dcolor; float* partials = A.partials;
    int* const s_tab32 = reinterpret_cast<int*>(s_tab64);
    __shared__ float s_wave[NW][4];
    __shared__ float s_max[NW];
    const int K = crf.K;
    for (int i = threadIdx.x; i < K - 1; i += NW * 64) s_tab64[i] = 0ull;
    const bool blur_hdr = (flags & HS_FLAG_BLUR_HDR) && N > 1;
    const float gs = blur_hdr ? 1.f : 1.f / (float)N;
    const float scale = (float)(K - 1) / (crf.umax - crf.umin);
    const int plane = plane_in;
    const int pose = plane / 3, ch = plane - 3 * pose;
    const int frame = blur_hdr ? pose : (A.F > 1 ? pose / N : 0);
    crf.dt = exposure[frame];
    const float* Hp = pose_hdr + ((int64_t)(blur_hdr ? A.F * N + frame : pose) * 3 + ch) * HW;
    const float* gp = dL_dcolor + ((int64_t)frame * 3 + ch) * HW;
    const float* t = crf.table + ch * K;
    const int lane = threadIdx.x & 63, wave = threadIdx.x >> 6;

    const int64_t i16 = ((int64_t)bxi * (NW * 64) + threadIdx.x) * 16;
    float Hv[16], g[16];
    if (i16 + 16 <= HW && (HW & 3) == 0) {
#pragma unroll
        for (int q = 0; q < 4; ++q) {
            const float4 h4 = reinterpret_cast<const float4*>(Hp + i16)[q];
            const float4 g4 = reinterpret_cast<const float4*>(gp + i16)[q];
            Hv[4 * q] = h4.x; Hv[4 * q + 1] = h4.y; Hv[4 * q + 2] = h4.z; Hv[4 * q + 3] = h4.w;
            g[4 * q] = g4.x * gs; g[4 * q + 1] = g4.y * gs; g[4 * q + 2] = g4.z * gs; g[4 * q + 3] = g4.w * gs;
        }
    } else {
#pragma unroll
        for (int e = 0; e < 16; ++e) {
            const bool ok = i16 + e < HW;
            Hv[e] = ok ? Hp[i16 + e] : 0.f;
            g[e] = ok ? gp[i16 + e] * gs : 0.f;
        }
    }
    float mx = 0.f;
#pragma unroll
    for (int e = 0; e < 16; ++e) mx = fmaxf(mx, fabsf(g[e]));
#pragma unroll
    for (int d = 32; d >= 1; d >>= 1) mx = fmaxf(mx, __shfl_xor(mx, d));
    if (lane == 0) s_max[wave] = mx;
    __syncthreads();
    mx = fmaxf(s_max[0], s_max[1]);
    if constexpr (NW == 4) mx = fmaxf(mx, fmaxf(s_max[2], s_max[3]));
    int xexp = 0;
    if (mx > 0.f && mx < 3.0e38f) (void)frexpf(mx, &xexp);
    const float to_fix = ldexpf(1.f, 19 - xexp), from_fix = ldexpf(1.f, xexp - 19);

    float gexp = 0.f, g_lo = 0.f, g_hi = 0.f;
    int run = -1;
    float r0 = 0.f, r1 = 0.f;
    auto flush = [&]() {
        atomicAdd(&s_tab32[2 * run], __float2int_rn(r0 * to_fix));
        atomicAdd(&s_tab32[2 * run + 1], __float2int_rn(r1 * to_fix));
    };
#pragma unroll
    for (int e = 0; e < 16; ++e) {
        int idx; float f, xv; bool in;
        crf_locate(crf, Hv[e], idx, f, xv, in);
        const bool lo = idx == 0 && f == 0.f, hi = idx == K - 2 && f == 1.f;
        g_lo += lo ? g[e] : 0.f;
        g_hi += hi ? g[e] : 0.f;
        if (!lo && !hi) {
            if (idx != run) {
                if (run >= 0) flush();
                run = idx; r0 = 0.f; r1 = 0.f;
            }
            r0 += (1.f - f) * g[e];
            r1 += f * g[e];
        }
        if (in) gexp += g[e] * (t[idx + 1] - t[idx]) * scale * __builtin_amdgcn_rcpf(xv) * Hv[e];
    }
    if (run >= 0) flush();
    gexp = wave_sum_hi(gexp);
    g_lo = wave_sum_hi(g_lo);
    g_hi = wave_sum_hi(g_hi);
    if (lane == 63) { s_wave[wave][0] = gexp; s_wave[wave][1] = g_lo; s_wave[wave][2] = g_hi; }
    __syncthreads();
    float* dst = partials + ((int64_t)plane_in * A.bx + bxi) * (K + 1);
    for (int k = threadIdx.x; k <= K; k += NW * 64) {
        float v;
        if (k == K) {
            v = NW == 4 ? ((s_wave[0][0] + s_wave[1][0]) + s_wave[2 % NW][0]) + s_wave[3 % NW][0] : s_wave[0][0] + s_wave[1][0];
        } else {
            long long acc = 0;
            if (k < K - 1) acc += (long long)s_tab32[2 * k];
            if (k > 0) acc += (long long)s_tab32[2 * (k - 1) + 1];
            v = (float)acc * from_fix;
            if (k == 0) v += NW == 4 ? ((s_wave[0][1] + s_wave[1][1]) + s_wave[2 % NW][1]) + s_wave[3 % NW][1] : s_wave[0][1] + s_wave[1][1];
            if (k == K - 1) v += NW == 4 ? ((s_wave[0][2] + s_wave[1][2]) + s_wave[2 % NW][2]) + s_wave[3 % NW][2] : s_wave[0][2] + s_wave[1][2];
        }
        dst[k] = v;
    }
}

struct RenderBwd {
    int W, H, gx, gy, ntiles, N, F, flags;
    const uint2* ranges; const uint32_t* point_list; const float4* rec; const float* bg;
    const float* final_T; const uint32_t* n_contrib; const float* pose_hdr;
    const float* dL_dcolor; const float* dL_dhdr; const float* dL_dalpha; const float* dL_dinvdepth;
    float4* pair_grads;
    uint8_t* pair_flags;
    const uint8_t* pair_act;
    Crf crf;
    const float* exposure;
    unsigned long long* stats;
    unsigned long long* timeline;
    uint32_t* queue;
    const uint32_t* tile_order;
    int grid_tiles;
    CrfGradArgs crf_tail;
};

__device__ __forceinline__ float pixel_grad(const RenderBwd& p, const Crf& c, int pose, int frame, int ch, int64_t pix, int64_t HW) {
    const float invN = 1.f / (float)p.N;
    const int64_t gpl = ((int64_t)frame * 3 + ch) * HW + pix;
    float g = p.dL_dcolor[gpl];
    if (!(p.flags & HS_FLAG_HDR)) return g * invN;
    float out = 0.f;
    if (p.N == 1 || !(p.flags & HS_FLAG_BLUR_HDR)) {
        const float Hv = p.pose_hdr[((int64_t)pose * 3 + ch) * HW + pix];
        out = crf_grad_H(c, ch, Hv, g * invN);
    } else {
        const float Hm = p.pose_hdr[((int64_t)(p.F * p.N + frame) * 3 + ch) * HW + pix];
        out = crf_grad_H(c, ch, Hm, g) * invN;
    }
    if (p.dL_dhdr) out += p.dL_dhdr[gpl] * invN;
    return out;
}

struct PixB {
    float T, dL0, dL1, dL2, q;
    float dLd;
    uint32_t last;
};

__device__ __forceinline__ void load_pixel_bwd(const RenderBwd& p, PixB& s, bool inside, int pose, int frame, int px, int py) {
    const int64_t HW = (int64_t)p.H * p.W;
    const int64_t pix = (int64_t)py * p.W + px;
    s.T = 0.f; s.dL0 = s.dL1 = s.dL2 = 0.f; s.last = 0;
    if (inside) {
        s.T = p.final_T[(int64_t)pose * HW + pix];
        s.last = p.n_contrib[(int64_t)pose * HW + pix];
        Crf c = p.crf;
        if (p.flags & HS_FLAG_HDR) c.dt = p.exposure[frame];
        s.dL0 = pixel_grad(p, c, pose, frame, 0, pix, HW);
        s.dL1 = pixel_grad(p, c, pose, frame, 1, pix, HW);
        s.dL2 = pixel_grad(p, c, pose, frame, 2, pix, HW);
    }
    float bg_dot = (p.bg[0] * s.dL0 + p.bg[1] * s.dL1) + p.bg[2] * s.dL2;
    if (p.dL_dalpha && inside) bg_dot -= p.dL_dalpha[pix] / (float)p.N;
    s.q = bg_dot;
    s.dLd = (p.dL_dinvdepth && inside) ? p.dL_dinvdepth[pix] / (float)p.N : 0.f;
}

struct PairB {
    f2 T, q, dL0, dL1, dL2, dLd;
};
__device__ __forceinline__ f2 splat(float v) { f2 r = {v, v}; return r; }
__device__ __forceinline__ PairB pack_pair(const PixB& a, const PixB& b) {
    PairB s;
    s.T = f2{a.T, b.T}; s.q = f2{a.q, b.q};
    s.dL0 = f2{a.dL0, b.dL0}; s.dL1 = f2{a.dL1, b.dL1}; s.dL2 = f2{a.dL2, b.dL2};
    s.dLd = f2{a.dLd, b.dLd};
    return s;
}
template <bool DEPTH>
__device__ __forceinline__ void step_bwd_pair(PairB& s, bool act0, bool act1, f2 G, f2 alpha, float o, float r, float g,
                                              float b, float invd, f2& sw, f2& dop, f2& dch) {
    const f2 ae = {act0 ? alpha.x : 0.f, act1 ? alpha.y : 0.f};
    const f2 one_m = splat(1.f) - ae;
    const f2 rcp = {__builtin_amdgcn_rcpf(one_m.x), __builtin_amdgcn_rcpf(one_m.y)};
    s.T *= rcp;
    dch = ae * s.T;
    f2 cd = (splat(r) * s.dL0 + pk_mul_hi(f2{r, g}, s.dL1)) + splat(b) * s.dL2;
    if constexpr (DEPTH) cd += splat(invd) * s.dLd;
    const f2 diff = cd - s.q;
    const f2 gd = G * (diff * s.T);
    s.q += ae * diff;
    dop = f2{act0 ? gd.x : 0.f, act1 ? gd.y : 0.f};
    sw = splat(o) * dop;
}

constexpr int kTailPct = 8;
constexpr int kAccF = 12;
constexpr int kBwdKB = 52;


template <bool DEPTH, bool STATS>
__global__ void __launch_bounds__(kBatch) __attribute__((amdgpu_waves_per_eu((DEPTH || STATS) ? 1 : 7)))
render_bwd_kernel(RenderBwd p) {
    constexpr int KB = kBwdKB;
    constexpr int NV = DEPTH ? 10 : 9;
    constexpr int kEntF = kAccF + 4 * NV;
    constexpr int kEntB = kEntF * 4;
    static_assert(kEntB % 16 == 0, "LDS entry records must stay 16-byte aligned");
    constexpr int kSentinel = KB * kEntB;
    constexpr int kListLen = KB + 8;
    __shared__ __attribute__((aligned(16))) float s_ent[(KB + 1) * kEntF];
    static_assert(KB * kEntF >= 2 * 7 * 128, "the pixel-state re-deal of the prologue borrows the staging area below the sentinel");
    __shared__ uint16_t s_list[2][2][kListLen];
    __shared__ uint8_t s_actb[kBatch];
    __shared__ uint32_t s_max[2];

    __shared__ uint32_t s_q;
    if constexpr (!STATS) {
        if ((int)blockIdx.x >= p.grid_tiles) {
            const int qd = (int)blockIdx.x - p.grid_tiles;
            crf_grad_body<2>(p.crf_tail, qd % p.crf_tail.bx, qd / p.crf_tail.bx, reinterpret_cast<unsigned long long*>(s_ent));
            return;
        }
    }
    const int n_tail = (int)((int64_t)p.grid_tiles * kTailPct / 100);
    const int n_static = p.grid_tiles - n_tail;
    if (threadIdx.x < kAccF) s_ent[KB * kEntF + threadIdx.x] = 0.f;
    for (;;) {
    int bidx = blockIdx.x;
    if ((int)blockIdx.x >= n_static) {
        __syncthreads();
        if (threadIdx.x == 0) {
            const uint32_t q = atomicAdd(p.queue, 1u);
            if (q == 2u * (uint32_t)n_tail - 1u) atomicExch(p.queue, 0u);
            s_q = q;
        }
        __syncthreads();
        if (s_q >= (uint32_t)n_tail) return;
        bidx = n_static + (int)s_q;
    }
    const int vt = p.tile_order ? (int)p.tile_order[bidx] : xcd_strip_tile(bidx, p.grid_tiles, p.gx);
    const int pose = vt / p.ntiles;
    const int tile = vt - pose * p.ntiles;
    const int tx = tile % p.gx, ty = tile / p.gx;
    const int wave = threadIdx.x >> 6, lane = threadIdx.x & 63;
    const int grp = lane >> 5;
    const int sx = tx * kTile, sy = ty * kTile + wave * 8;
    int px, py0;
    lane_pixels(lane, sx, sy, px, py0);
    const int py1 = py0 + 1;
    const float pxf = (float)px;
    const f2 pyf = {(float)py0, (float)py1};

    unsigned long long t_start = 0;
    if constexpr (STATS) t_start = wall_clock64();
    const uint2 range = p.ranges[vt];

    PixB s0, s1;
    {
        const int qx = sx + (lane & 15), qy0 = sy + 2 * (lane >> 4);
        PixB t0, t1;
        const int frame = p.F > 1 ? pose / p.N : 0;
        load_pixel_bwd(p, t0, qx < p.W && qy0 < p.H, pose, frame, qx, qy0);
        load_pixel_bwd(p, t1, qx < p.W && qy0 + 1 < p.H, pose, frame, qx, qy0 + 1);
        float* const o = s_ent + wave * (7 * 128);
        const int r0 = (qy0 - sy) * 16 + (lane & 15), r1 = r0 + 16;
        o[r0] = t0.T; o[r1] = t1.T;
        o[128 + r0] = t0.dL0; o[128 + r1] = t1.dL0;
        o[256 + r0] = t0.dL1; o[256 + r1] = t1.dL1;
        o[384 + r0] = t0.dL2; o[384 + r1] = t1.dL2;
        o[512 + r0] = t0.q; o[512 + r1] = t1.q;
        o[640 + r0] = t0.dLd; o[640 + r1] = t1.dLd;
        o[768 + r0] = __uint_as_float(t0.last); o[768 + r1] = __uint_as_float(t1.last);
        __builtin_amdgcn_fence(__ATOMIC_RELEASE, "wavefront");
        __builtin_amdgcn_wave_barrier();
        const int p0 = (py0 - sy) * 16 + (px - sx), p1 = p0 + 16;
        s0.T = o[p0]; s0.dL0 = o[128 + p0]; s0.dL1 = o[256 + p0]; s0.dL2 = o[384 + p0]; s0.q = o[512 + p0];
        s0.dLd = o[640 + p0]; s0.last = __float_as_uint(o[768 + p0]);
        s1.T = o[p1]; s1.dL0 = o[128 + p1]; s1.dL1 = o[256 + p1]; s1.dL2 = o[384 + p1]; s1.q = o[512 + p1];
        s1.dLd = o[640 + p1]; s1.last = __float_as_uint(o[768 + p1]);
    }
    PairB ps = pack_pair(s0, s1);

    const uint32_t wave_max = wave_max_u32(max(s0.last, s1.last));
    if (lane == 0) s_max[wave] = wave_max;
    __syncthreads();
    const int n_proc = (int)max(s_max[0], s_max[1]);

    int red_off = -1;
    const bool red_t0 = (lane & 3) == 0;
    {
        const int row = lane >> 4, k = (lane & 15) >> 2;
        constexpr int kOrd[4] = {0, 2, 1, 3};
        if ((lane & 3) == 0) red_off = ((row & 1) ? 4 : 0) + kOrd[k];
        else if ((lane & 3) == 1 && !(row & 1) && k == 0) red_off = 8;
        else if (DEPTH && (lane & 3) == 1 && !(row & 1) && k == 2) red_off = 9;
        if (red_off >= 0) red_off = (kAccF + NV * (2 * grp + wave) + red_off) * 4;
    }
    const int xor16_addr = (lane ^ 16) << 2;
    char* const ent = reinterpret_cast<char*>(s_ent);
    float* const my_ent = s_ent + threadIdx.x * kEntF;
    const uint16_t* const my_list = s_list[wave][grp];
    WaveStats ws;
    if constexpr (STATS) ws.clear();
    const int nb = (n_proc + KB - 1) / KB;
    uint32_t id_next = 0, act_next = 0;
    if (nb > 0) {
        const int base = (nb - 1) * KB;
        if ((int)threadIdx.x < n_proc - base) {
            id_next = p.point_list[range.x + base + threadIdx.x];
            act_next = p.pair_act[(int64_t)range.x + base + threadIdx.x];
        }
    }
    for (int bi = nb - 1; bi >= 0; --bi) {
        const int base = bi * KB;
        const int cnt = min(KB, n_proc - base);
        if constexpr (STATS) { if (wave == 0) { ws.v[kStBwdStaged] += cnt; ws.v[kStBwdBatches] += 1; } }
        __syncthreads();
        const bool taken = (int)threadIdx.x < cnt && act_next != 0;
        s_actb[threadIdx.x] = (uint8_t)((int)threadIdx.x < cnt ? act_next : 0u);
        if (taken) {
            const float4* r = p.rec + kRecF4 * (int64_t)id_next;
            float4 ra = r[0], rb = r[1];
            float4 rc = r[2];
            if constexpr (DEPTH) rc.y = 1.f / rc.y;
            scale_entry(ra, rb);
            reinterpret_cast<float4*>(my_ent)[0] = ra;
            reinterpret_cast<float4*>(my_ent)[1] = rb;
            reinterpret_cast<float4*>(my_ent)[2] = rc;
        }
        if (bi > 0 && (int)threadIdx.x < KB) {
            id_next = p.point_list[range.x + base - KB + threadIdx.x];
            act_next = p.pair_act[(int64_t)range.x + base - KB + threadIdx.x];
        }
        __syncthreads();
        {
            int maxn = 0;
#pragma unroll
            for (int g = 0; g < 2; ++g) {
                const uint32_t gbit = 1u << (2 * g + wave);
                uint16_t* lst = s_list[wave][g];
                int n_g = 0;
#pragma unroll
                for (int k = (KB + 63) / 64 - 1; k >= 0; --k) {
                    const uint64_t m = __ballot((s_actb[k * 64 + lane] & gbit) != 0);
                    const int c = __popcll(m);
                    if ((m >> lane) & 1ull) lst[n_g + c - 1 - mask_prefix(m)] = (uint16_t)((k * 64 + lane) * kEntB);
                    n_g += c;
                }
#pragma unroll
                for (int t = lane; t < kListLen; t += 64)
                    if (t >= n_g) lst[t] = (uint16_t)kSentinel;
                maxn = max(maxn, n_g);
            }
            if constexpr (STATS) {
                const uint32_t wbits = 5u << wave;
                uint32_t mine = 0;
#pragma unroll
                for (int k = 0; k < (KB + 63) / 64; ++k) mine += __popcll(__ballot((s_actb[k * 64 + lane] & wbits) != 0));
                ws.v[kStBwdCulled] += (uint32_t)cnt - mine;
            }
            const int lim0 = ((int)s0.last - base) * kEntB, lim1 = ((int)s1.last - base) * kEntB;
            int jb = (int)my_list[0];
            for (int ti = 0; ti < maxn; ++ti) {
                int jn = (int)my_list[ti + 1];
                asm("" : "+v"(jn));
                const float4 a = *reinterpret_cast<const float4*>(ent + jb);
                const float4 b = *reinterpret_cast<const float4*>(ent + jb + 16);
                const float2 c = *reinterpret_cast<const float2*>(ent + jb + 32);
                const float cb = c.x;
                const float invd = DEPTH ? c.y : 0.f;
                const float dx = a.x - pxf;
                const f2 dy = a.y - pyf;
                const float t = a.z * dx * dx, u = a.w * dx;
                const f2 pw = dy * (b.x * dy + u) + t;
                const float G0 = hs_exp2(pw.x), G1 = hs_exp2(pw.y);
                const float al0 = fminf(kAlphaMax, b.y * G0), al1 = fminf(kAlphaMax, b.y * G1);
                const bool act0 = (jb < lim0) && (pw.x <= 0.f) && (al0 >= kAlphaMin);
                const bool act1 = (jb < lim1) && (pw.y <= 0.f) && (al1 >= kAlphaMin);
                if constexpr (STATS) {
                    const int lanes = __popcll(__ballot(act0 || act1));
                    ws.v[kStBwdTrips] += 1;
                    ws.v[kStBwdEmpty] += lanes == 0;
                    ws.v[kStBwdActivePix] += __popcll(__ballot(act0)) + __popcll(__ballot(act1));
                    const int bin = lanes == 0 ? 0 : lanes <= 4 ? 1 : lanes <= 8 ? 2 : lanes <= 16 ? 3 : lanes <= 32 ? 4 : 5;
                    ws.v[kStBwdHist + bin] += 1;
                }
                f2 sw, dop, dch;
                step_bwd_pair<DEPTH>(ps, act0, act1, f2{G0, G1}, f2{al0, al1}, b.y, b.z, b.w, cb, invd, sw, dop, dch);
                const f2 m = sw * dy;
                const f2 m2 = m * dy;
                const f2 c0 = dch * ps.dL0, c1 = dch * ps.dL1, c2 = dch * ps.dL2;
                float g[9];
                g[0] = (sw.x + sw.y) * dx;
                g[1] = m.x + m.y;
                g[2] = g[0] * dx;
                g[3] = g[1] * dx;
                g[4] = m2.x + m2.y;
                g[5] = dop.x + dop.y;
                g[6] = c0.x + c0.y;
                g[7] = c1.x + c1.y;
                g[8] = c2.x + c2.y;
                float g9 = 0.f;
                if constexpr (DEPTH) {
                    const f2 cd = dch * ps.dLd;
                    g9 = cd.x + cd.y;
                }
                float t0, t1;
                group_reduce<DEPTH>(g, g9, xor16_addr, t0, t1);
                if (red_off >= 0) *reinterpret_cast<float*>(ent + jb + red_off) = red_t0 ? t0 : t1;
                jb = jn;
            }
        }
        __syncthreads();
        if (taken) {
            float v[10] = {0.f, 0.f, 0.f, 0.f, 0.f, 0.f, 0.f, 0.f, 0.f, 0.f};
            const uint32_t ab = s_actb[threadIdx.x];
#pragma unroll
            for (int pl = 0; pl < 4; ++pl) {
                const bool on = (ab >> pl) & 1u;
#pragma unroll
                for (int q = 0; q < NV; ++q) {
                    const float x = my_ent[kAccF + NV * pl + q];
                    v[q] += on ? x : 0.f;
                }
            }
            const float4 a = reinterpret_cast<const float4*>(my_ent)[0];
            const float4 c = reinterpret_cast<const float4*>(my_ent)[2];
            const float A = a.z * (-2.f / kLog2e), B = a.w * (-1.f / kLog2e), C = my_ent[4] * (-2.f / kLog2e);
            const float ddelx_dx = 0.5f * (float)p.W, ddely_dy = 0.5f * (float)p.H;
            const float gmx = -(A * v[0] + B * v[1]) * ddelx_dx;
            const float gmy = -(C * v[1] + B * v[0]) * ddely_dy;
            const int rad = __float_as_int(c.z);
            const uint32_t off = __float_as_uint(c.w);
            const int rminx = min(p.gx, max(0, (int)((a.x - (float)rad) / (float)kTile)));
            const int rminy = min(p.gy, max(0, (int)((a.y - (float)rad) / (float)kTile)));
            const int rmaxx = min(p.gx, max(0, (int)((a.x + (float)rad + (float)(kTile - 1)) / (float)kTile)));
            const int64_t slot = (int64_t)off + (int64_t)(ty - rminy) * (rmaxx - rminx) + (tx - rminx);
            p.pair_flags[slot] = 1;
            float4* o = p.pair_grads + kPairF4 * slot;
            o[0] = make_float4(gmx, gmy, -0.5f * v[2], -v[3]);
            o[1] = make_float4(-0.5f * v[4], v[5], v[6], v[7]);
            o[2] = make_float4(v[8], v[9], 0.f, 0.f);
            if constexpr (kPairF4 == 4) o[3] = make_float4(0.f, 0.f, 0.f, 0.f);
        }
    }
    if constexpr (STATS) {
        ws.flush(p.stats);
        if (p.timeline && threadIdx.x == 0) {
            p.timeline[3 * bidx + 0] = t_start;
            p.timeline[3 * bidx + 1] = wall_clock64();
            const uint32_t xcc = __builtin_amdgcn_s_getreg((3 << 11) | (0 << 6) | 20);
            const uint32_t hw = __builtin_amdgcn_s_getreg((31 << 11) | (0 << 6) | 4);
            p.timeline[3 * bidx + 2] = ((unsigned long long)xcc << 32) | hw;
        }
    }
    if ((int)blockIdx.x < n_static) return;
    }
}

__global__ void __launch_bounds__(256) crf_grad_kernel(CrfGradArgs A) {
    extern __shared__ unsigned long long s_crf_tab[];
    crf_grad_body<4>(A, (int)blockIdx.x, (int)blockIdx.y, s_crf_tab);
}

__global__ void __launch_bounds__(256) crf_reduce_kernel(CrfReduce c) { crf_reduce_block(c, (int)blockIdx.x); }

}

static bool orders_tiles(int grid) { return grid <= 6 * 3072; }


int launch_render_fwd(const hs_fwd_args& a, const hs_layout& L, hipStream_t s, unsigned long long* stats) {
    const hs_dims& d = a.dims;
    RenderFwd p;
    p.W = d.W; p.H = d.H; p.gx = (d.W + kTile - 1) / kTile;
    const int gy = (d.H + kTile - 1) / kTile;
    const int F = frames_of(d);
    p.ntiles = p.gx * gy; p.N = d.n_poses / F; p.flags = a.flags;
    char* bin = (char*)a.binning; char* img = (char*)a.image; char* geom = (char*)a.geom;
    p.ranges = (const uint2*)(bin + L.ranges); p.point_list = (const uint32_t*)(bin + L.point_list);
    p.rec = (const float4*)(geom + L.rec); p.bg = a.bg;
    p.out_color = a.out_color; p.out_hdr = a.out_hdr;
    p.final_T = (float*)(img + L.final_T); p.n_contrib = (uint32_t*)(img + L.n_contrib);
    const bool need_pose = (a.flags & HS_FLAG_HDR) || p.N > 1;
    p.pose_hdr = need_pose ? (float*)(img + L.pose_hdr) : nullptr;
    p.crf.table = a.crf_table; p.crf.K = a.crf_K; p.crf.umin = a.crf_umin; p.crf.umax = a.crf_umax; p.crf.dt = 1.f;
    p.exposure = a.exposure;
    p.out_invdepth = a.out_invdepth;
    p.stats = stats; p.timeline = nullptr;
    p.pair_act = (uint8_t*)bin + L.pair_act;
    p.tile_work = (uint32_t*)(img + L.tile_work);
    const int grid = p.ntiles * d.n_poses;
    if (stats) {
        if (a.out_invdepth) render_fwd_kernel<true, true><<<grid, kBatch, 0, s>>>(p);
        else render_fwd_kernel<false, true><<<grid, kBatch, 0, s>>>(p);
    } else if (a.out_invdepth) render_fwd_kernel<true, false><<<grid, kBatch, 0, s>>>(p);
    else render_fwd_kernel<false, false><<<grid, kBatch, 0, s>>>(p);
    HS_LAUNCH_CHECK();
    if (orders_tiles(grid)) {
        const int n_static = grid - (int)((int64_t)grid * kTailPct / 100);
        order_tiles_kernel<<<8, 1024, 0, s>>>(grid, p.gx, n_static, p.tile_work, (uint32_t*)(img + L.tile_order));
        HS_LAUNCH_CHECK();
    }
    if (p.N > 1) {
        const int64_t HW = (int64_t)d.W * d.H;
        resolve_kernel<<<ceil_div((int64_t)F * 3 * HW, 256), 256, 0, s>>>(HW, p.N, F, a.flags, p.pose_hdr, p.crf, a.exposure,
                                                                         a.out_color, a.out_hdr);
        HS_LAUNCH_CHECK();
    }
    return HS_OK;
}

static bool crf_grad_args(const hs_bwd_args& a, const hs_layout& L, CrfGradArgs& A, int waves = 4) {
    const hs_dims& d = a.dims;
    if (!((a.flags & HS_FLAG_HDR) && (a.dL_dcrf_table || a.dL_dexposure))) return false;
    A.crf.table = a.crf_table; A.crf.K = a.crf_K; A.crf.umin = a.crf_umin; A.crf.umax = a.crf_umax; A.crf.dt = 1.f;
    A.HW = (int64_t)d.W * d.H; A.F = frames_of(d); A.N = d.n_poses / A.F; A.flags = a.flags;
    A.partials = (float*)((char*)a.bwd + L.crf_partials);
    A.pose_hdr = (const float*)((const char*)a.image + L.pose_hdr);
    A.exposure = a.exposure; A.dL_dcolor = a.dL_dout_color;
    const bool blur_hdr = (a.flags & HS_FLAG_BLUR_HDR) && A.N > 1;
    A.planes = 3 * (blur_hdr ? A.F : d.n_poses);
    A.bx = ceil_div(A.HW, (int64_t)waves * kCrfPixPerWave);
    return true;
}

int launch_crf_bwd(const hs_bwd_args& a, const hs_layout& L, hipStream_t s, CrfReduce* defer, bool in_render_tail) {
    CrfGradArgs A;
    if (!crf_grad_args(a, L, A, in_render_tail ? 2 : 4)) return HS_OK;
    if (!in_render_tail)
        crf_grad_kernel<<<dim3(A.bx, A.planes), 256, (size_t)(a.crf_K - 1) * sizeof(unsigned long long), s>>>(A);
    CrfReduce cr;
    cr.partials = A.partials; cr.bx = A.bx; cr.planes = A.planes; cr.K = a.crf_K; cr.d_table = a.dL_dcrf_table;
    cr.F = A.F;
    cr.d_exposure = a.dL_dexposure; cr.nblocks = ceil_div(3 * a.crf_K + cr.F, 4);
    if (defer) *defer = cr;
    else crf_reduce_kernel<<<cr.nblocks, 256, 0, s>>>(cr);
    HS_LAUNCH_CHECK();
    return HS_OK;
}

int launch_render_bwd(const hs_bwd_args& a, const hs_layout& L, hipStream_t s, unsigned long long* stats,
                      unsigned long long* timeline, bool crf_in_tail) {
    const hs_dims& d = a.dims;
    RenderBwd p;
    p.W = d.W; p.H = d.H; p.gx = (d.W + kTile - 1) / kTile; p.gy = (d.H + kTile - 1) / kTile;
    p.F = frames_of(d);
    p.ntiles = p.gx * p.gy; p.N = d.n_poses / p.F; p.flags = a.flags;
    const char* bin = (const char*)a.binning; const char* img = (const char*)a.image; const char* geom = (const char*)a.geom;
    p.ranges = (const uint2*)(bin + L.ranges); p.point_list = (const uint32_t*)(bin + L.point_list);
    p.rec = (const float4*)(geom + L.rec); p.bg = a.bg;
    p.final_T = (const float*)(img + L.final_T); p.n_contrib = (const uint32_t*)(img + L.n_contrib);
    p.pose_hdr = (const float*)(img + L.pose_hdr);
    p.dL_dcolor = a.dL_dout_color; p.dL_dhdr = a.dL_dout_hdr; p.dL_dalpha = a.dL_dout_alpha;
    p.dL_dinvdepth = a.dL_dout_invdepth;
    p.pair_grads = (float4*)((char*)a.bwd + L.pair_grads);
    p.crf.table = a.crf_table; p.crf.K = a.crf_K; p.crf.umin = a.crf_umin; p.crf.umax = a.crf_umax; p.crf.dt = 1.f;
    p.exposure = a.exposure;
    p.pair_flags = (uint8_t*)a.binning + L.pair_flags;
    p.pair_act = (const uint8_t*)a.binning + L.pair_act;
    p.stats = stats; p.timeline = timeline;
    p.queue = &((hs_counters*)((char*)a.geom + L.counters))->reserved[3];
    p.tile_order = orders_tiles(p.ntiles * d.n_poses) ? (const uint32_t*)(img + L.tile_order) : nullptr;
    int grid = p.ntiles * d.n_poses;
    p.grid_tiles = grid;
    if (crf_in_tail && !stats && crf_grad_args(a, L, p.crf_tail, 2)) grid += p.crf_tail.bx * p.crf_tail.planes;
    if (stats) {
        if (a.dL_dout_invdepth) render_bwd_kernel<true, true><<<grid, kBatch, 0, s>>>(p);
        else render_bwd_kernel<false, true><<<grid, kBatch, 0, s>>>(p);
    } else if (a.dL_dout_invdepth) render_bwd_kernel<true, false><<<grid, kBatch, 0, s>>>(p);
    else render_bwd_kernel<false, false><<<grid, kBatch, 0, s>>>(p);
    HS_LAUNCH_CHECK();
    return HS_OK;
}

int render_stats_count() { return kStCount; }

int64_t crf_partial_floats(int K, int64_t HW, int n_poses) {
    return K > 0 ? (int64_t)ceil_div(HW, 2 * kCrfPixPerWave) * 3 * n_poses * (K + 1) : 0;
}

}
```

Before: 960.8 images/s.

## Run render backward as one-wave workgroups with four pixels per lane

Restructures the render backward kernel to launch 64-thread workgroups (one wave) instead of the 256-thread batch. Each lane now handles two pixel pairs (A/B rows), so per-Gaussian gradient terms are summed in registers before a single DPP row/quad reduction that replaces the permlane/bpermute group reduction. The CRF gradient tail body gains an NH parameter so a one-wave block can process several pieces in turn, and the knot limit for running CRF in the render tail is now derived from the staging buffer size. The goal is to cut cross-wave LDS traffic and barriers and to amortize Gaussian loads over more pixels. The cost is higher register pressure per lane and a smaller shared staging buffer.

```diff
diff --git a/casualhdrsplat_amd/csrc/api.hip b/casualhdrsplat_amd/csrc/api.hip
--- a/casualhdrsplat_amd/csrc/api.hip
+++ b/casualhdrsplat_amd/csrc/api.hip
@@ -355,7 +355,7 @@
     }
     if (a->dims.P == 0) return HS_OK;
     const bool crf_in_tail = HS_TUNE_CRF_IN_RENDER_TAIL && (a->stages & HS_BWD_RENDER) && (a->stages & HS_BWD_CRF) &&
-                             !(a->flags & HS_FLAG_DEBUG) && a->crf_K <= 1024;
+                             !(a->flags & HS_FLAG_DEBUG) && a->crf_K <= render_bwd_tail_max_knots();
     if (a->stages & HS_BWD_RENDER) {
         rc = launch_render_bwd(*a, L, s, nullptr, nullptr, crf_in_tail);
         if (rc) return rc;
diff --git a/casualhdrsplat_amd/csrc/hs_common.h b/casualhdrsplat_amd/csrc/hs_common.h
--- a/casualhdrsplat_amd/csrc/hs_common.h
+++ b/casualhdrsplat_amd/csrc/hs_common.h
@@ -71,6 +71,7 @@
 int launch_render_bwd(const hs_bwd_args& a, const hs_layout& L, hipStream_t s, unsigned long long* stats = nullptr,
                       unsigned long long* timeline = nullptr, bool crf_in_tail = false);
 int render_stats_count();
+int render_bwd_tail_max_knots();
 struct CrfReduce;
 int launch_crf_bwd(const hs_bwd_args& a, const hs_layout& L, hipStream_t s, CrfReduce* defer, bool in_render_tail = false);
 int launch_preprocess_bwd(const hs_bwd_args& a, const hs_layout& L, hipStream_t s, bool segsum, bool project,
diff --git a/casualhdrsplat_amd/csrc/render.hip b/casualhdrsplat_amd/csrc/render.hip
--- a/casualhdrsplat_amd/csrc/render.hip
+++ b/casualhdrsplat_amd/csrc/render.hip
@@ -49,72 +49,60 @@
     v += dpp<0x143, 0xC>(v);
     return v;
 }
-__device__ __forceinline__ float halve16(float x, float y) {
-    auto r = __builtin_amdgcn_permlane16_swap(__float_as_uint(x), __float_as_uint(y), false, false);
-    return __uint_as_float(r[0]) + __uint_as_float(r[1]);
-}
 template <bool TEN>
-__device__ __forceinline__ void reduce_in_rows(const float* g, float g9, float& w0, float& w1, float& w2) {
+__device__ __forceinline__ void row_reduce(const float* g, float g9, float& t0, float& t1, float& t2) {
     float z0, z1, z2, z3, z4;
     if constexpr (TEN) {
         asm("s_nop 1\n\t"
-            "v_add_f32_dpp %3, %9, %9 row_shr:8 row_mask:0xf bank_mask:0xc\n\t"
-            "v_add_f32_dpp %3, %8, %8 row_shl:8 row_mask:0xf bank_mask:0x3\n\t"
-            "v_add_f32_dpp %4, %11, %11 row_shr:8 row_mask:0xf bank_mask:0xc\n\t"
-            "v_add_f32_dpp %4, %10, %10 row_shl:8 row_mask:0xf bank_mask:0x3\n\t"
-            "v_add_f32_dpp %5, %13, %13 row_shr:8 row_mask:0xf bank_mask:0xc\n\t"
-            "v_add_f32_dpp %5, %12, %12 row_shl:8 row_mask:0xf bank_mask:0x3\n\t"
-            "v_add_f32_dpp %6, %15, %15 row_shr:8 row_mask:0xf bank_mask:0xc\n\t"
-            "v_add_f32_dpp %6, %14, %14 row_shl:8 row_mask:0xf bank_mask:0x3\n\t"
-            "v_add_f32_dpp %7, %17, %17 row_shr:8 row_mask:0xf bank_mask:0xc\n\t"
-            "v_add_f32_dpp %7, %16, %16 row_shl:8 row_mask:0xf bank_mask:0x3\n\t"
-            "v_add_f32_dpp %0, %4, %4 row_shr:4 row_mask:0xf bank_mask:0xa\n\t"
-            "v_add_f32_dpp %0, %3, %3 row_shl:4 row_mask:0xf bank_mask:0x5\n\t"
-            "v_add_f32_dpp %1, %6, %6 row_shr:4 row_mask:0xf bank_mask:0xa\n\t"
-            "v_add_f32_dpp %1, %5, %5 row_shl:4 row_mask:0xf bank_mask:0x5\n\t"
-            "v_add_f32_dpp %2, %7, %7 row_shr:4 row_mask:0xf bank_mask:0xa\n\t"
-            "v_add_f32_dpp %2, %7, %7 row_shl:4 row_mask:0xf bank_mask:0x5\n\t"
-            "s_nop 1"
-            : "=&v"(w0), "=&v"(w1), "=&v"(w2), "=&v"(z0), "=&v"(z1), "=&v"(z2), "=&v"(z3), "=&v"(z4)
+            "v_add_f32_dpp %3, %9, %9 row_shr:4 row_mask:0xf bank_mask:0xa\n\t"
+            "v_add_f32_dpp %3, %8, %8 row_shl:4 row_mask:0xf bank_mask:0x5\n\t"
+            "v_add_f32_dpp %4, %11, %11 row_shr:4 row_mask:0xf bank_mask:0xa\n\t"
+            "v_add_f32_dpp %4, %10, %10 row_shl:4 row_mask:0xf bank_mask:0x5\n\t"
+            "v_add_f32_dpp %5, %13, %13 row_shr:4 row_mask:0xf bank_mask:0xa\n\t"
+            "v_add_f32_dpp %5, %12, %12 row_shl:4 row_mask:0xf bank_mask:0x5\n\t"
+            "v_add_f32_dpp %6, %15, %15 row_shr:4 row_mask:0xf bank_mask:0xa\n\t"
+            "v_add_f32_dpp %6, %14, %14 row_shl:4 row_mask:0xf bank_mask:0x5\n\t"
+            "v_add_f32_dpp %7, %17, %17 row_shr:4 row_mask:0xf bank_mask:0xa\n\t"
+            "v_add_f32_dpp %7, %16, %16 row_shl:4 row_mask:0xf bank_mask:0x5\n\t"
+            "v_add_f32_dpp %0, %4, %4 row_shr:8 row_mask:0xf bank_mask:0xc\n\t"
+            "v_add_f32_dpp %0, %3, %3 row_shl:8 row_mask:0xf bank_mask:0x3\n\t"
+            "v_add_f32_dpp %1, %6, %6 row_shr:8 row_mask:0xf bank_mask:0xc\n\t"
+            "v_add_f32_dpp %1, %5, %5 row_shl:8 row_mask:0xf bank_mask:0x3\n\t"
+            "v_add_f32_dpp %2, %7, %7 row_shr:8 row_mask:0xf bank_mask:0xc\n\t"
+            "v_add_f32_dpp %2, %7, %7 row_shl:8 row_mask:0xf bank_mask:0x3\n\t"
+            "v_add_f32_dpp %0, %0, %0 quad_perm:[1,0,3,2] row_mask:0xf bank_mask:0xf\n\t"
+            "v_add_f32_dpp %1, %1, %1 quad_perm:[1,0,3,2] row_mask:0xf bank_mask:0xf\n\t"
+            "v_add_f32_dpp %2, %2, %2 quad_perm:[1,0,3,2] row_mask:0xf bank_mask:0xf\n\t"
+            "v_add_f32_dpp %0, %0, %0 quad_perm:[2,3,0,1] row_mask:0xf bank_mask:0xf\n\t"
+            "v_add_f32_dpp %1, %1, %1 quad_perm:[2,3,0,1] row_mask:0xf bank_mask:0xf\n\t"
+            "v_add_f32_dpp %2, %2, %2 quad_perm:[2,3,0,1] row_mask:0xf bank_mask:0xf"
+            : "=&v"(t0), "=&v"(t1), "=&v"(t2), "=&v"(z0), "=&v"(z1), "=&v"(z2), "=&v"(z3), "=&v"(z4)
             : "v"(g[0]), "v"(g[1]), "v"(g[2]), "v"(g[3]), "v"(g[4]), "v"(g[5]), "v"(g[6]), "v"(g[7]), "v"(g[8]), "v"(g9));
     } else {
         asm("s_nop 1\n\t"
-            "v_add_f32_dpp %3, %9, %9 row_shr:8 row_mask:0xf bank_mask:0xc\n\t"
-            "v_add_f32_dpp %3, %8, %8 row_shl:8 row_mask:0xf bank_mask:0x3\n\t"
-            "v_add_f32_dpp %4, %11, %11 row_shr:8 row_mask:0xf bank_mask:0xc\n\t"
-            "v_add_f32_dpp %4, %10, %10 row_shl:8 row_mask:0xf bank_mask:0x3\n\t"
-            "v_add_f32_dpp %5, %13, %13 row_shr:8 row_mask:0xf bank_mask:0xc\n\t"
-            "v_add_f32_dpp %5, %12, %12 row_shl:8 row_mask:0xf bank_mask:0x3\n\t"
-            "v_add_f32_dpp %6, %15, %15 row_shr:8 row_mask:0xf bank_mask:0xc\n\t"
-            "v_add_f32_dpp %6, %14, %14 row_shl:8 row_mask:0xf bank_mask:0x3\n\t"
-            "v_add_f32_dpp %7, %16, %16 row_ror:8 row_mask:0xf bank_mask:0xf\n\t"
-            "v_add_f32_dpp %0, %4, %4 row_shr:4 row_mask:0xf bank_mask:0xa\n\t"
-            "v_add_f32_dpp %0, %3, %3 row_shl:4 row_mask:0xf bank_mask:0x5\n\t"
-            "v_add_f32_dpp %1, %6, %6 row_shr:4 row_mask:0xf bank_mask:0xa\n\t"
-            "v_add_f32_dpp %1, %5, %5 row_shl:4 row_mask:0xf bank_mask:0x5\n\t"
-            "v_add_f32_dpp %2, %7, %7 row_ror:4 row_mask:0xf bank_mask:0xf\n\t"
-            "s_nop 1"
-            : "=&v"(w0), "=&v"(w1), "=&v"(w2), "=&v"(z0), "=&v"(z1), "=&v"(z2), "=&v"(z3), "=&v"(z4)
+            "v_add_f32_dpp %3, %9, %9 row_shr:4 row_mask:0xf bank_mask:0xa\n\t"
+            "v_add_f32_dpp %3, %8, %8 row_shl:4 row_mask:0xf bank_mask:0x5\n\t"
+            "v_add_f32_dpp %4, %11, %11 row_shr:4 row_mask:0xf bank_mask:0xa\n\t"
+            "v_add_f32_dpp %4, %10, %10 row_shl:4 row_mask:0xf bank_mask:0x5\n\t"
+            "v_add_f32_dpp %5, %13, %13 row_shr:4 row_mask:0xf bank_mask:0xa\n\t"
+            "v_add_f32_dpp %5, %12, %12 row_shl:4 row_mask:0xf bank_mask:0x5\n\t"
+            "v_add_f32_dpp %6, %15, %15 row_shr:4 row_mask:0xf bank_mask:0xa\n\t"
+            "v_add_f32_dpp %6, %14, %14 row_shl:4 row_mask:0xf bank_mask:0x5\n\t"
+            "v_add_f32_dpp %7, %16, %16 row_ror:4 row_mask:0xf bank_mask:0xf\n\t"
+            "v_add_f32_dpp %0, %4, %4 row_shr:8 row_mask:0xf bank_mask:0xc\n\t"
+            "v_add_f32_dpp %0, %3, %3 row_shl:8 row_mask:0xf bank_mask:0x3\n\t"
+            "v_add_f32_dpp %1, %6, %6 row_shr:8 row_mask:0xf bank_mask:0xc\n\t"
+            "v_add_f32_dpp %1, %5, %5 row_shl:8 row_mask:0xf bank_mask:0x3\n\t"
+            "v_add_f32_dpp %2, %7, %7 row_ror:8 row_mask:0xf bank_mask:0xf\n\t"
+            "v_add_f32_dpp %0, %0, %0 quad_perm:[1,0,3,2] row_mask:0xf bank_mask:0xf\n\t"
+            "v_add_f32_dpp %1, %1, %1 quad_perm:[1,0,3,2] row_mask:0xf bank_mask:0xf\n\t"
+            "v_add_f32_dpp %2, %2, %2 quad_perm:[1,0,3,2] row_mask:0xf bank_mask:0xf\n\t"
+            "v_add_f32_dpp %0, %0, %0 quad_perm:[2,3,0,1] row_mask:0xf bank_mask:0xf\n\t"
+            "v_add_f32_dpp %1, %1, %1 quad_perm:[2,3,0,1] row_mask:0xf bank_mask:0xf\n\t"
+            "v_add_f32_dpp %2, %2, %2 quad_perm:[2,3,0,1] row_mask:0xf bank_mask:0xf"
+            : "=&v"(t0), "=&v"(t1), "=&v"(t2), "=&v"(z0), "=&v"(z1), "=&v"(z2), "=&v"(z3), "=&v"(z4)
             : "v"(g[0]), "v"(g[1]), "v"(g[2]), "v"(g[3]), "v"(g[4]), "v"(g[5]), "v"(g[6]), "v"(g[7]), "v"(g[8]));
     }
-}
-__device__ __forceinline__ float reduce_in_quads(float t) {
-    asm("s_nop 1\n\t"
-        "v_add_f32_dpp %0, %0, %0 quad_perm:[1,0,3,2] row_mask:0xf bank_mask:0xf\n\t"
-        "s_nop 1\n\t"
-        "v_add_f32_dpp %0, %0, %0 quad_perm:[2,3,0,1] row_mask:0xf bank_mask:0xf"
-        : "+v"(t));
-    return t;
-}
-
-template <bool TEN>
-__device__ __forceinline__ void group_reduce(const float* g, float g9, int xor16_addr, float& t0, float& t1) {
-    float w0, w1, w2;
-    reduce_in_rows<TEN>(g, g9, w0, w1, w2);
-    const float u0 = halve16(w0, w1);
-    const float u1 = w2 + __int_as_float(__builtin_amdgcn_ds_bpermute(xor16_addr, __float_as_int(w2)));
-    t0 = reduce_in_quads(u0);
-    t1 = reduce_in_quads(u1);
 }
 
 __device__ __forceinline__ int mask_prefix(uint64_t m) {
@@ -602,13 +590,16 @@
     int bx, planes;
 };
 
-template <int NW>
+template <int NW, int NH = 1>
 __device__ __forceinline__ void crf_grad_body(const CrfGradArgs& A, const int bxi, const int plane_in,
                                               unsigned long long* const s_tab64) {
+    static_assert(NH == 1 || NW == 1, "pieces in turn: one-wave workgroups only");
+    constexpr int NP = NW * NH;
+    static_assert(NP == 2 || NP == 4, "the pieces' float sums are added in a stated order");
     const int64_t HW = A.HW; const int N = A.N, flags = A.flags; const float* pose_hdr = A.pose_hdr; Crf crf = A.crf;
     const float* exposure = A.exposure; const float* dL_dcolor = A.dL_dcolor; float* partials = A.partials;
     int* const s_tab32 = reinterpret_cast<int*>(s_tab64);
-    __shared__ float s_wave[NW][4];
+    __shared__ float s_wave[NP][4];
     __shared__ float s_max[NW];
     const int K = crf.K;
     for (int i = threadIdx.x; i < K - 1; i += NW * 64) s_tab64[i] = 0ull;
@@ -624,79 +615,93 @@
     const float* t = crf.table + ch * K;
     const int lane = threadIdx.x & 63, wave = threadIdx.x >> 6;
 
-    const int64_t i16 = ((int64_t)bxi * (NW * 64) + threadIdx.x) * 16;
-    float Hv[16], g[16];
-    if (i16 + 16 <= HW && (HW & 3) == 0) {
-#pragma unroll
-        for (int q = 0; q < 4; ++q) {
-            const float4 h4 = reinterpret_cast<const float4*>(Hp + i16)[q];
-            const float4 g4 = reinterpret_cast<const float4*>(gp + i16)[q];
-            Hv[4 * q] = h4.x; Hv[4 * q + 1] = h4.y; Hv[4 * q + 2] = h4.z; Hv[4 * q + 3] = h4.w;
-            g[4 * q] = g4.x * gs; g[4 * q + 1] = g4.y * gs; g[4 * q + 2] = g4.z * gs; g[4 * q + 3] = g4.w * gs;
-        }
-    } else {
-#pragma unroll
-        for (int e = 0; e < 16; ++e) {
-            const bool ok = i16 + e < HW;
-            Hv[e] = ok ? Hp[i16 + e] : 0.f;
-            g[e] = ok ? gp[i16 + e] * gs : 0.f;
+    float Hv[NH][16], g[NH][16];
+#pragma unroll
+    for (int h = 0; h < NH; ++h) {
+        const int64_t i16 = ((int64_t)bxi * (NP * 64) + h * 64 + threadIdx.x) * 16;
+        if (i16 + 16 <= HW && (HW & 3) == 0) {
+#pragma unroll
+            for (int q = 0; q < 4; ++q) {
+                const float4 h4 = reinterpret_cast<const float4*>(Hp + i16)[q];
+                const float4 g4 = reinterpret_cast<const float4*>(gp + i16)[q];
+                Hv[h][4 * q] = h4.x; Hv[h][4 * q + 1] = h4.y; Hv[h][4 * q + 2] = h4.z; Hv[h][4 * q + 3] = h4.w;
+                g[h][4 * q] = g4.x * gs; g[h][4 * q + 1] = g4.y * gs; g[h][4 * q + 2] = g4.z * gs; g[h][4 * q + 3] = g4.w * gs;
+            }
+        } else {
+#pragma unroll
+            for (int e = 0; e < 16; ++e) {
+                const bool ok = i16 + e < HW;
+                Hv[h][e] = ok ? Hp[i16 + e] : 0.f;
+                g[h][e] = ok ? gp[i16 + e] * gs : 0.f;
+            }
         }
     }
     float mx = 0.f;
 #pragma unroll
-    for (int e = 0; e < 16; ++e) mx = fmaxf(mx, fabsf(g[e]));
+    for (int h = 0; h < NH; ++h)
+#pragma unroll
+        for (int e = 0; e < 16; ++e) mx = fmaxf(mx, fabsf(g[h][e]));
 #pragma unroll
     for (int d = 32; d >= 1; d >>= 1) mx = fmaxf(mx, __shfl_xor(mx, d));
     if (lane == 0) s_max[wave] = mx;
     __syncthreads();
-    mx = fmaxf(s_max[0], s_max[1]);
-    if constexpr (NW == 4) mx = fmaxf(mx, fmaxf(s_max[2], s_max[3]));
+    mx = s_max[0];
+    if constexpr (NW >= 2) mx = fmaxf(mx, s_max[1 % NW]);
+    if constexpr (NW == 4) mx = fmaxf(mx, fmaxf(s_max[2 % NW], s_max[3 % NW]));
     int xexp = 0;
     if (mx > 0.f && mx < 3.0e38f) (void)frexpf(mx, &xexp);
     const float to_fix = ldexpf(1.f, 19 - xexp), from_fix = ldexpf(1.f, xexp - 19);
 
-    float gexp = 0.f, g_lo = 0.f, g_hi = 0.f;
-    int run = -1;
-    float r0 = 0.f, r1 = 0.f;
-    auto flush = [&]() {
-        atomicAdd(&s_tab32[2 * run], __float2int_rn(r0 * to_fix));
-        atomicAdd(&s_tab32[2 * run + 1], __float2int_rn(r1 * to_fix));
+#pragma unroll
+    for (int h = 0; h < NH; ++h) {
+        float gexp = 0.f, g_lo = 0.f, g_hi = 0.f;
+        int run = -1;
+        float r0 = 0.f, r1 = 0.f;
+        auto flush = [&]() {
+            atomicAdd(&s_tab32[2 * run], __float2int_rn(r0 * to_fix));
+            atomicAdd(&s_tab32[2 * run + 1], __float2int_rn(r1 * to_fix));
+        };
+#pragma unroll
+        for (int e = 0; e < 16; ++e) {
+            int idx; float f, xv; bool in;
+            crf_locate(crf, Hv[h][e], idx, f, xv, in);
+            const bool lo = idx == 0 && f == 0.f, hi = idx == K - 2 && f == 1.f;
+            g_lo += lo ? g[h][e] : 0.f;
+            g_hi += hi ? g[h][e] : 0.f;
+            if (!lo && !hi) {
+                if (idx != run) {
+                    if (run >= 0) flush();
+                    run = idx; r0 = 0.f; r1 = 0.f;
+                }
+                r0 += (1.f - f) * g[h][e];
+                r1 += f * g[h][e];
+            }
+            if (in) gexp += g[h][e] * (t[idx + 1] - t[idx]) * scale * __builtin_amdgcn_rcpf(xv) * Hv[h][e];
+        }
+        if (run >= 0) flush();
+        gexp = wave_sum_hi(gexp);
+        g_lo = wave_sum_hi(g_lo);
+        g_hi = wave_sum_hi(g_hi);
+        if (lane == 63) { s_wave[wave + h][0] = gexp; s_wave[wave + h][1] = g_lo; s_wave[wave + h][2] = g_hi; }
+    }
+    __syncthreads();
+    auto pieces = [&](int c) {
+        float v = s_wave[0][c] + s_wave[1][c];
+        if constexpr (NP == 4) v = (v + s_wave[2 % NP][c]) + s_wave[3 % NP][c];
+        return v;
     };
-#pragma unroll
-    for (int e = 0; e < 16; ++e) {
-        int idx; float f, xv; bool in;
-        crf_locate(crf, Hv[e], idx, f, xv, in);
-        const bool lo = idx == 0 && f == 0.f, hi = idx == K - 2 && f == 1.f;
-        g_lo += lo ? g[e] : 0.f;
-        g_hi += hi ? g[e] : 0.f;
-        if (!lo && !hi) {
-            if (idx != run) {
-                if (run >= 0) flush();
-                run = idx; r0 = 0.f; r1 = 0.f;
-            }
-            r0 += (1.f - f) * g[e];
-            r1 += f * g[e];
-        }
-        if (in) gexp += g[e] * (t[idx + 1] - t[idx]) * scale * __builtin_amdgcn_rcpf(xv) * Hv[e];
-    }
-    if (run >= 0) flush();
-    gexp = wave_sum_hi(gexp);
-    g_lo = wave_sum_hi(g_lo);
-    g_hi = wave_sum_hi(g_hi);
-    if (lane == 63) { s_wave[wave][0] = gexp; s_wave[wave][1] = g_lo; s_wave[wave][2] = g_hi; }
-    __syncthreads();
     float* dst = partials + ((int64_t)plane_in * A.bx + bxi) * (K + 1);
     for (int k = threadIdx.x; k <= K; k += NW * 64) {
         float v;
         if (k == K) {
-            v = NW == 4 ? ((s_wave[0][0] + s_wave[1][0]) + s_wave[2 % NW][0]) + s_wave[3 % NW][0] : s_wave[0][0] + s_wave[1][0];
+            v = pieces(0);
         } else {
             long long acc = 0;
             if (k < K - 1) acc += (long long)s_tab32[2 * k];
             if (k > 0) acc += (long long)s_tab32[2 * (k - 1) + 1];
             v = (float)acc * from_fix;
-            if (k == 0) v += NW == 4 ? ((s_wave[0][1] + s_wave[1][1]) + s_wave[2 % NW][1]) + s_wave[3 % NW][1] : s_wave[0][1] + s_wave[1][1];
-            if (k == K - 1) v += NW == 4 ? ((s_wave[0][2] + s_wave[1][2]) + s_wave[2 % NW][2]) + s_wave[3 % NW][2] : s_wave[0][2] + s_wave[1][2];
+            if (k == 0) v += pieces(1);
+            if (k == K - 1) v += pieces(2);
         }
         dst[k] = v;
     }
@@ -792,129 +797,138 @@
 
 constexpr int kTailPct = 8;
 constexpr int kAccF = 12;
-constexpr int kBwdKB = 52;
-
+constexpr int kBwdWave = 64;
+#ifndef HS_TUNE_BWD_KB
+#define HS_TUNE_BWD_KB 48
+#endif
+#ifndef HS_TUNE_BWD_WAVES
+#define HS_TUNE_BWD_WAVES 4
+#endif
+constexpr int kBwdKB = HS_TUNE_BWD_KB;
+constexpr int bwd_stage_floats(int ent_f) { return (kBwdKB + 1) * ent_f > 7 * 256 ? (kBwdKB + 1) * ent_f : 7 * 256; }
+
+__device__ __forceinline__ void lane_pixels4(int lane, int sx, int sy, int& px, int& py0) {
+    const int blk = lane >> 4;
+    px = sx + 8 * (blk & 1) + (lane & 7);
+    py0 = sy + 8 * (blk >> 1) + 4 * ((lane >> 3) & 1);
+}
 
 template <bool DEPTH, bool STATS>
-__global__ void __launch_bounds__(kBatch) __attribute__((amdgpu_waves_per_eu((DEPTH || STATS) ? 1 : 7)))
+__global__ void __launch_bounds__(kBwdWave) __attribute__((amdgpu_waves_per_eu((DEPTH || STATS) ? 1 : HS_TUNE_BWD_WAVES)))
 render_bwd_kernel(RenderBwd p) {
     constexpr int KB = kBwdKB;
     constexpr int NV = DEPTH ? 10 : 9;
     constexpr int kEntF = kAccF + 4 * NV;
     constexpr int kEntB = kEntF * 4;
     static_assert(kEntB % 16 == 0, "LDS entry records must stay 16-byte aligned");
+    static_assert(KB <= kBwdWave, "one staged entry per lane, one ballot per list");
     constexpr int kSentinel = KB * kEntB;
     constexpr int kListLen = KB + 8;
-    __shared__ __attribute__((aligned(16))) float s_ent[(KB + 1) * kEntF];
-    static_assert(KB * kEntF >= 2 * 7 * 128, "the pixel-state re-deal of the prologue borrows the staging area below the sentinel");
-    __shared__ uint16_t s_list[2][2][kListLen];
-    __shared__ uint8_t s_actb[kBatch];
-    __shared__ uint32_t s_max[2];
-
-    __shared__ uint32_t s_q;
+    constexpr int kStageF = bwd_stage_floats(kEntF);
+    __shared__ __attribute__((aligned(16))) float s_ent[kStageF];
+    __shared__ uint16_t s_list[4][kListLen];
+
+    const int lane = threadIdx.x;
     if constexpr (!STATS) {
         if ((int)blockIdx.x >= p.grid_tiles) {
             const int qd = (int)blockIdx.x - p.grid_tiles;
-            crf_grad_body<2>(p.crf_tail, qd % p.crf_tail.bx, qd / p.crf_tail.bx, reinterpret_cast<unsigned long long*>(s_ent));
+            crf_grad_body<1, 2>(p.crf_tail, qd % p.crf_tail.bx, qd / p.crf_tail.bx, reinterpret_cast<unsigned long long*>(s_ent));
             return;
         }
     }
     const int n_tail = (int)((int64_t)p.grid_tiles * kTailPct / 100);
     const int n_static = p.grid_tiles - n_tail;
-    if (threadIdx.x < kAccF) s_ent[KB * kEntF + threadIdx.x] = 0.f;
     for (;;) {
     int bidx = blockIdx.x;
     if ((int)blockIdx.x >= n_static) {
-        __syncthreads();
-        if (threadIdx.x == 0) {
-            const uint32_t q = atomicAdd(p.queue, 1u);
+        uint32_t q = 0;
+        if (lane == 0) {
+            q = atomicAdd(p.queue, 1u);
             if (q == 2u * (uint32_t)n_tail - 1u) atomicExch(p.queue, 0u);
-            s_q = q;
-        }
-        __syncthreads();
-        if (s_q >= (uint32_t)n_tail) return;
-        bidx = n_static + (int)s_q;
+        }
+        q = __builtin_amdgcn_readfirstlane(q);
+        if (q >= (uint32_t)n_tail) return;
+        bidx = n_static + (int)q;
     }
     const int vt = p.tile_order ? (int)p.tile_order[bidx] : xcd_strip_tile(bidx, p.grid_tiles, p.gx);
     const int pose = vt / p.ntiles;
     const int tile = vt - pose * p.ntiles;
     const int tx = tile % p.gx, ty = tile / p.gx;
-    const int wave = threadIdx.x >> 6, lane = threadIdx.x & 63;
-    const int grp = lane >> 5;
-    const int sx = tx * kTile, sy = ty * kTile + wave * 8;
+    const int blk = lane >> 4;
+    const int plane = 2 * (blk & 1) + (blk >> 1);
+    const int sx = tx * kTile, sy = ty * kTile;
     int px, py0;
-    lane_pixels(lane, sx, sy, px, py0);
-    const int py1 = py0 + 1;
+    lane_pixels4(lane, sx, sy, px, py0);
     const float pxf = (float)px;
-    const f2 pyf = {(float)py0, (float)py1};
+    const f2 pyfA = {(float)py0, (float)(py0 + 1)}, pyfB = {(float)(py0 + 2), (float)(py0 + 3)};
 
     unsigned long long t_start = 0;
     if constexpr (STATS) t_start = wall_clock64();
     const uint2 range = p.ranges[vt];
 
-    PixB s0, s1;
+    PairB psA, psB;
+    uint32_t last0, last1, last2, last3;
     {
-        const int qx = sx + (lane & 15), qy0 = sy + 2 * (lane >> 4);
-        PixB t0, t1;
+        __syncthreads();
+        const int qc = lane & 15, qr = lane >> 4;
         const int frame = p.F > 1 ? pose / p.N : 0;
-        load_pixel_bwd(p, t0, qx < p.W && qy0 < p.H, pose, frame, qx, qy0);
-        load_pixel_bwd(p, t1, qx < p.W && qy0 + 1 < p.H, pose, frame, qx, qy0 + 1);
-        float* const o = s_ent + wave * (7 * 128);
-        const int r0 = (qy0 - sy) * 16 + (lane & 15), r1 = r0 + 16;
-        o[r0] = t0.T; o[r1] = t1.T;
-        o[128 + r0] = t0.dL0; o[128 + r1] = t1.dL0;
-        o[256 + r0] = t0.dL1; o[256 + r1] = t1.dL1;
-        o[384 + r0] = t0.dL2; o[384 + r1] = t1.dL2;
-        o[512 + r0] = t0.q; o[512 + r1] = t1.q;
-        o[640 + r0] = t0.dLd; o[640 + r1] = t1.dLd;
-        o[768 + r0] = __uint_as_float(t0.last); o[768 + r1] = __uint_as_float(t1.last);
-        __builtin_amdgcn_fence(__ATOMIC_RELEASE, "wavefront");
-        __builtin_amdgcn_wave_barrier();
-        const int p0 = (py0 - sy) * 16 + (px - sx), p1 = p0 + 16;
-        s0.T = o[p0]; s0.dL0 = o[128 + p0]; s0.dL1 = o[256 + p0]; s0.dL2 = o[384 + p0]; s0.q = o[512 + p0];
-        s0.dLd = o[640 + p0]; s0.last = __float_as_uint(o[768 + p0]);
-        s1.T = o[p1]; s1.dL0 = o[128 + p1]; s1.dL1 = o[256 + p1]; s1.dL2 = o[384 + p1]; s1.q = o[512 + p1];
-        s1.dLd = o[640 + p1]; s1.last = __float_as_uint(o[768 + p1]);
-    }
-    PairB ps = pack_pair(s0, s1);
-
-    const uint32_t wave_max = wave_max_u32(max(s0.last, s1.last));
-    if (lane == 0) s_max[wave] = wave_max;
-    __syncthreads();
-    const int n_proc = (int)max(s_max[0], s_max[1]);
+        float* const o = s_ent;
+#pragma unroll
+        for (int k = 0; k < 4; ++k) {
+            const int row = qr + 4 * k;
+            PixB t;
+            load_pixel_bwd(p, t, sx + qc < p.W && sy + row < p.H, pose, frame, sx + qc, sy + row);
+            const int r = row * 16 + qc;
+            o[r] = t.T; o[256 + r] = t.dL0; o[512 + r] = t.dL1; o[768 + r] = t.dL2; o[1024 + r] = t.q;
+            o[1280 + r] = t.dLd; o[1536 + r] = __uint_as_float(t.last);
+        }
+        __syncthreads();
+        const float* const m = o + (py0 - sy) * 16 + (px - sx);
+        psA.T = f2{m[0], m[16]};                  psB.T = f2{m[32], m[48]};
+        psA.dL0 = f2{m[256], m[256 + 16]};        psB.dL0 = f2{m[256 + 32], m[256 + 48]};
+        psA.dL1 = f2{m[512], m[512 + 16]};        psB.dL1 = f2{m[512 + 32], m[512 + 48]};
+        psA.dL2 = f2{m[768], m[768 + 16]};        psB.dL2 = f2{m[768 + 32], m[768 + 48]};
+        psA.q = f2{m[1024], m[1024 + 16]};        psB.q = f2{m[1024 + 32], m[1024 + 48]};
+        psA.dLd = f2{m[1280], m[1280 + 16]};      psB.dLd = f2{m[1280 + 32], m[1280 + 48]};
+        last0 = __float_as_uint(m[1536]); last1 = __float_as_uint(m[1536 + 16]);
+        last2 = __float_as_uint(m[1536 + 32]); last3 = __float_as_uint(m[1536 + 48]);
+        __syncthreads();
+        if (lane < kAccF) s_ent[KB * kEntF + lane] = 0.f;
+    }
+
+    const int n_proc = (int)__builtin_amdgcn_readfirstlane(wave_max_u32(max(max(last0, last1), max(last2, last3))));
 
     int red_off = -1;
-    const bool red_t0 = (lane & 3) == 0;
+    const int red_j = lane & 3;
     {
-        const int row = lane >> 4, k = (lane & 15) >> 2;
-        constexpr int kOrd[4] = {0, 2, 1, 3};
-        if ((lane & 3) == 0) red_off = ((row & 1) ? 4 : 0) + kOrd[k];
-        else if ((lane & 3) == 1 && !(row & 1) && k == 0) red_off = 8;
-        else if (DEPTH && (lane & 3) == 1 && !(row & 1) && k == 2) red_off = 9;
-        if (red_off >= 0) red_off = (kAccF + NV * (2 * grp + wave) + red_off) * 4;
-    }
-    const int xor16_addr = (lane ^ 16) << 2;
+        const int k = (lane & 15) >> 2;
+        if (red_j == 0) red_off = k;
+        else if (red_j == 1) red_off = 4 + k;
+        else if (red_j == 2 && k == 0) red_off = 8;
+        else if (DEPTH && red_j == 2 && k == 1) red_off = 9;
+        if (red_off >= 0) red_off = (kAccF + NV * plane + red_off) * 4;
+    }
     char* const ent = reinterpret_cast<char*>(s_ent);
-    float* const my_ent = s_ent + threadIdx.x * kEntF;
-    const uint16_t* const my_list = s_list[wave][grp];
+    float* const my_ent = s_ent + lane * kEntF;
+    const uint16_t* const my_list = s_list[blk];
     WaveStats ws;
     if constexpr (STATS) ws.clear();
     const int nb = (n_proc + KB - 1) / KB;
     uint32_t id_next = 0, act_next = 0;
     if (nb > 0) {
         const int base = (nb - 1) * KB;
-        if ((int)threadIdx.x < n_proc - base) {
-            id_next = p.point_list[range.x + base + threadIdx.x];
-            act_next = p.pair_act[(int64_t)range.x + base + threadIdx.x];
+        if (lane < n_proc - base) {
+            id_next = p.point_list[range.x + base + lane];
+            act_next = p.pair_act[(int64_t)range.x + base + lane];
         }
     }
     for (int bi = nb - 1; bi >= 0; --bi) {
         const int base = bi * KB;
         const int cnt = min(KB, n_proc - base);
-        if constexpr (STATS) { if (wave == 0) { ws.v[kStBwdStaged] += cnt; ws.v[kStBwdBatches] += 1; } }
+        if constexpr (STATS) { ws.v[kStBwdStaged] += cnt; ws.v[kStBwdBatches] += 1; }
         __syncthreads();
-        const bool taken = (int)threadIdx.x < cnt && act_next != 0;
-        s_actb[threadIdx.x] = (uint8_t)((int)threadIdx.x < cnt ? act_next : 0u);
+        const uint32_t act = lane < cnt ? act_next : 0u;
+        const bool taken = act != 0;
         if (taken) {
             const float4* r = p.rec + kRecF4 * (int64_t)id_next;
             float4 ra = r[0], rb = r[1];
@@ -925,40 +939,33 @@
             reinterpret_cast<float4*>(my_ent)[1] = rb;
             reinterpret_cast<float4*>(my_ent)[2] = rc;
         }
-        if (bi > 0 && (int)threadIdx.x < KB) {
-            id_next = p.point_list[range.x + base - KB + threadIdx.x];
-            act_next = p.pair_act[(int64_t)range.x + base - KB + threadIdx.x];
-        }
-        __syncthreads();
+        if (bi > 0 && lane < KB) {
+            id_next = p.point_list[range.x + base - KB + lane];
+            act_next = p.pair_act[(int64_t)range.x + base - KB + lane];
+        }
         {
             int maxn = 0;
-#pragma unroll
-            for (int g = 0; g < 2; ++g) {
-                const uint32_t gbit = 1u << (2 * g + wave);
-                uint16_t* lst = s_list[wave][g];
-                int n_g = 0;
-#pragma unroll
-                for (int k = (KB + 63) / 64 - 1; k >= 0; --k) {
-                    const uint64_t m = __ballot((s_actb[k * 64 + lane] & gbit) != 0);
-                    const int c = __popcll(m);
-                    if ((m >> lane) & 1ull) lst[n_g + c - 1 - mask_prefix(m)] = (uint16_t)((k * 64 + lane) * kEntB);
-                    n_g += c;
-                }
+            [[maybe_unused]] int n_half[2] = {0, 0};
+#pragma unroll
+            for (int b = 0; b < 4; ++b) {
+                const uint32_t gbit = 1u << (2 * (b & 1) + (b >> 1));
+                uint16_t* lst = s_list[b];
+                const uint64_t m = __ballot((act & gbit) != 0);
+                const int c = __popcll(m);
+                if ((m >> lane) & 1ull) lst[c - 1 - mask_prefix(m)] = (uint16_t)(lane * kEntB);
 #pragma unroll
                 for (int t = lane; t < kListLen; t += 64)
-                    if (t >= n_g) lst[t] = (uint16_t)kSentinel;
-                maxn = max(maxn, n_g);
+                    if (t >= c) lst[t] = (uint16_t)kSentinel;
+                maxn = max(maxn, c);
+                n_half[b >> 1] = max(n_half[b >> 1], c);
             }
-            if constexpr (STATS) {
-                const uint32_t wbits = 5u << wave;
-                uint32_t mine = 0;
-#pragma unroll
-                for (int k = 0; k < (KB + 63) / 64; ++k) mine += __popcll(__ballot((s_actb[k * 64 + lane] & wbits) != 0));
-                ws.v[kStBwdCulled] += (uint32_t)cnt - mine;
-            }
-            const int lim0 = ((int)s0.last - base) * kEntB, lim1 = ((int)s1.last - base) * kEntB;
+            if constexpr (STATS) ws.v[kStBwdCulled] += (uint32_t)cnt - (uint32_t)__popcll(__ballot(taken));
+            __syncthreads();
+            const int lim0 = ((int)last0 - base) * kEntB, lim1 = ((int)last1 - base) * kEntB;
+            const int lim2 = ((int)last2 - base) * kEntB, lim3 = ((int)last3 - base) * kEntB;
             int jb = (int)my_list[0];
-            for (int ti = 0; ti < maxn; ++ti) {
+            const int n_it = __builtin_amdgcn_readfirstlane(maxn);
+            for (int ti = 0; ti < n_it; ++ti) {
                 int jn = (int)my_list[ti + 1];
                 asm("" : "+v"(jn));
                 const float4 a = *reinterpret_cast<const float4*>(ent + jb);
@@ -967,54 +974,68 @@
                 const float cb = c.x;
                 const float invd = DEPTH ? c.y : 0.f;
                 const float dx = a.x - pxf;
-                const f2 dy = a.y - pyf;
+                const f2 dyA = a.y - pyfA, dyB = a.y - pyfB;
                 const float t = a.z * dx * dx, u = a.w * dx;
-                const f2 pw = dy * (b.x * dy + u) + t;
-                const float G0 = hs_exp2(pw.x), G1 = hs_exp2(pw.y);
+                const f2 pwA = dyA * (b.x * dyA + u) + t, pwB = dyB * (b.x * dyB + u) + t;
+                const float G0 = hs_exp2(pwA.x), G1 = hs_exp2(pwA.y), G2 = hs_exp2(pwB.x), G3 = hs_exp2(pwB.y);
                 const float al0 = fminf(kAlphaMax, b.y * G0), al1 = fminf(kAlphaMax, b.y * G1);
-                const bool act0 = (jb < lim0) && (pw.x <= 0.f) && (al0 >= kAlphaMin);
-                const bool act1 = (jb < lim1) && (pw.y <= 0.f) && (al1 >= kAlphaMin);
+                const float al2 = fminf(kAlphaMax, b.y * G2), al3 = fminf(kAlphaMax, b.y * G3);
+                const bool act0 = (jb < lim0) && (pwA.x <= 0.f) && (al0 >= kAlphaMin);
+                const bool act1 = (jb < lim1) && (pwA.y <= 0.f) && (al1 >= kAlphaMin);
+                const bool act2 = (jb < lim2) && (pwB.x <= 0.f) && (al2 >= kAlphaMin);
+                const bool act3 = (jb < lim3) && (pwB.y <= 0.f) && (al3 >= kAlphaMin);
                 if constexpr (STATS) {
-                    const int lanes = __popcll(__ballot(act0 || act1));
-                    ws.v[kStBwdTrips] += 1;
-                    ws.v[kStBwdEmpty] += lanes == 0;
-                    ws.v[kStBwdActivePix] += __popcll(__ballot(act0)) + __popcll(__ballot(act1));
-                    const int bin = lanes == 0 ? 0 : lanes <= 4 ? 1 : lanes <= 8 ? 2 : lanes <= 16 ? 3 : lanes <= 32 ? 4 : 5;
-                    ws.v[kStBwdHist + bin] += 1;
+                    const uint64_t lanes = __ballot(act0 || act1 || act2 || act3);
+#pragma unroll
+                    for (int h = 0; h < 2; ++h) {
+                        if (ti < n_half[h]) {
+                            const int nl = __popc((uint32_t)(lanes >> (32 * h)));
+                            ws.v[kStBwdTrips] += 1;
+                            ws.v[kStBwdEmpty] += nl == 0;
+                            const int bin = nl == 0 ? 0 : nl <= 4 ? 1 : nl <= 8 ? 2 : nl <= 16 ? 3 : nl <= 32 ? 4 : 5;
+                            ws.v[kStBwdHist + bin] += 1;
+                        }
+                    }
+                    ws.v[kStBwdActivePix] += __popcll(__ballot(act0)) + __popcll(__ballot(act1)) + __popcll(__ballot(act2)) +
+                                             __popcll(__ballot(act3));
                 }
-                f2 sw, dop, dch;
-                step_bwd_pair<DEPTH>(ps, act0, act1, f2{G0, G1}, f2{al0, al1}, b.y, b.z, b.w, cb, invd, sw, dop, dch);
-                const f2 m = sw * dy;
-                const f2 m2 = m * dy;
-                const f2 c0 = dch * ps.dL0, c1 = dch * ps.dL1, c2 = dch * ps.dL2;
+                f2 swA, dopA, dchA, swB, dopB, dchB;
+                step_bwd_pair<DEPTH>(psA, act0, act1, f2{G0, G1}, f2{al0, al1}, b.y, b.z, b.w, cb, invd, swA, dopA, dchA);
+                step_bwd_pair<DEPTH>(psB, act2, act3, f2{G2, G3}, f2{al2, al3}, b.y, b.z, b.w, cb, invd, swB, dopB, dchB);
+                const f2 sw = swA + swB;
+                const f2 mA = swA * dyA, mB = swB * dyB;
+                const f2 m = mA + mB;
+                const f2 m2 = mA * dyA + mB * dyB;
+                const f2 c0 = dchA * psA.dL0 + dchB * psB.dL0;
+                const f2 c1 = dchA * psA.dL1 + dchB * psB.dL1;
+                const f2 c2 = dchA * psA.dL2 + dchB * psB.dL2;
                 float g[9];
                 g[0] = (sw.x + sw.y) * dx;
                 g[1] = m.x + m.y;
                 g[2] = g[0] * dx;
                 g[3] = g[1] * dx;
                 g[4] = m2.x + m2.y;
-                g[5] = dop.x + dop.y;
+                g[5] = (dopA.x + dopA.y) + (dopB.x + dopB.y);
                 g[6] = c0.x + c0.y;
                 g[7] = c1.x + c1.y;
                 g[8] = c2.x + c2.y;
                 float g9 = 0.f;
                 if constexpr (DEPTH) {
-                    const f2 cd = dch * ps.dLd;
+                    const f2 cd = dchA * psA.dLd + dchB * psB.dLd;
                     g9 = cd.x + cd.y;
                 }
-                float t0, t1;
-                group_reduce<DEPTH>(g, g9, xor16_addr, t0, t1);
-                if (red_off >= 0) *reinterpret_cast<float*>(ent + jb + red_off) = red_t0 ? t0 : t1;
+                float t0, t1, t2;
+                row_reduce<DEPTH>(g, g9, t0, t1, t2);
+                if (red_off >= 0) *reinterpret_cast<float*>(ent + jb + red_off) = red_j == 0 ? t0 : red_j == 1 ? t1 : t2;
                 jb = jn;
             }
         }
         __syncthreads();
         if (taken) {
             float v[10] = {0.f, 0.f, 0.f, 0.f, 0.f, 0.f, 0.f, 0.f, 0.f, 0.f};
-            const uint32_t ab = s_actb[threadIdx.x];
 #pragma unroll
             for (int pl = 0; pl < 4; ++pl) {
-                const bool on = (ab >> pl) & 1u;
+                const bool on = (act >> pl) & 1u;
 #pragma unroll
                 for (int q = 0; q < NV; ++q) {
                     const float x = my_ent[kAccF + NV * pl + q];
@@ -1037,13 +1058,15 @@
             float4* o = p.pair_grads + kPairF4 * slot;
             o[0] = make_float4(gmx, gmy, -0.5f * v[2], -v[3]);
             o[1] = make_float4(-0.5f * v[4], v[5], v[6], v[7]);
-            o[2] = make_float4(v[8], v[9], 0.f, 0.f);
-            if constexpr (kPairF4 == 4) o[3] = make_float4(0.f, 0.f, 0.f, 0.f);
+            float zero = 0.f;
+            asm volatile("" : "+v"(zero));
+            o[2] = make_float4(v[8], v[9], zero, zero);
+            if constexpr (kPairF4 == 4) o[3] = make_float4(zero, zero, zero, zero);
         }
     }
     if constexpr (STATS) {
         ws.flush(p.stats);
-        if (p.timeline && threadIdx.x == 0) {
+        if (p.timeline && lane == 0) {
             p.timeline[3 * bidx + 0] = t_start;
             p.timeline[3 * bidx + 1] = wall_clock64();
             const uint32_t xcc = __builtin_amdgcn_s_getreg((3 << 11) | (0 << 6) | 20);
@@ -1163,16 +1186,18 @@
     p.grid_tiles = grid;
     if (crf_in_tail && !stats && crf_grad_args(a, L, p.crf_tail, 2)) grid += p.crf_tail.bx * p.crf_tail.planes;
     if (stats) {
-        if (a.dL_dout_invdepth) render_bwd_kernel<true, true><<<grid, kBatch, 0, s>>>(p);
-        else render_bwd_kernel<false, true><<<grid, kBatch, 0, s>>>(p);
-    } else if (a.dL_dout_invdepth) render_bwd_kernel<true, false><<<grid, kBatch, 0, s>>>(p);
-    else render_bwd_kernel<false, false><<<grid, kBatch, 0, s>>>(p);
+        if (a.dL_dout_invdepth) render_bwd_kernel<true, true><<<grid, kBwdWave, 0, s>>>(p);
+        else render_bwd_kernel<false, true><<<grid, kBwdWave, 0, s>>>(p);
+    } else if (a.dL_dout_invdepth) render_bwd_kernel<true, false><<<grid, kBwdWave, 0, s>>>(p);
+    else render_bwd_kernel<false, false><<<grid, kBwdWave, 0, s>>>(p);
     HS_LAUNCH_CHECK();
     return HS_OK;
 }
 
 int render_stats_count() { return kStCount; }
 
+int render_bwd_tail_max_knots() { return bwd_stage_floats(kAccF + 4 * 9) / 2 + 1; }
+
 int64_t crf_partial_floats(int K, int64_t HW, int n_poses) {
     return K > 0 ? (int64_t)ceil_div(HW, 2 * kCrfPixPerWave) * 3 * n_poses * (K + 1) : 0;
 }
```

Result: faster. 983.4 images/s, median of 6 (+2.4%).
